# jopohl/urh

Hardware: AMD Instinct MI355X
Metric: Msamples/s IQ->bits (1 GiB complex64 2-FSK per GPU, qad materialised, compact outputs copied to the host) (higher is better)
Workload: dtype f32

## Files before the change

include/urhgpu.h:

```cpp
#ifndef URHGPU_H
#define URHGPU_H

#include <stdint.h>

#ifdef __cplusplus
extern "C" {
#endif

#define URHGPU_VERSION 100

#define URHGPU_OK 0
#define URHGPU_ERR_HIP (-1)
#define URHGPU_ERR_DTYPE (-2)
#define URHGPU_ERR_ARG (-3)
#define URHGPU_ERR_CAPACITY (-4)
#define URHGPU_ERR_UNSUPPORTED (-5)
#define URHGPU_ERR_NO_DEVICE (-6)

#define URHGPU_DT_I8 0
#define URHGPU_DT_U8 1
#define URHGPU_DT_I16 2
#define URHGPU_DT_U16 3
#define URHGPU_DT_F32 4

// ... 216 lines not shown
int urhgpu_msg_divisor_histogram(const uint64_t *lens, int64_t n, uint64_t *hist_out, int64_t cap, int64_t *hist_len, int64_t *tol_out);
int urhgpu_bit_length_from_order(const uint64_t *hist, const int64_t *order_desc, int64_t len, int64_t *bitlen_out);

int urhgpu_minmax(urhgpu_ctx *ctx, const void *arr, int dtype, int64_t n, void *out2);
int urhgpu_segment_messages(urhgpu_ctx *ctx, const void *magnitudes, int is_f64, int64_t n, float noise_threshold, int64_t *seg_out,
                            int64_t cap_seg, int64_t *n_seg);
int urhgpu_get_plateau_lengths(urhgpu_ctx *ctx, const float *rect_data, int64_t n, float center, int percentage, uint64_t *out, int64_t cap,
                               int64_t *n_out);
int urhgpu_threshold_divisor_histogram(const uint64_t *lens, int64_t n, float threshold, uint64_t *hist_out, int64_t cap, int64_t *hist_len);
int urhgpu_median_filter(urhgpu_ctx *ctx, const double *data, int64_t n, unsigned int k, float *out);

int urhgpu_test_fast_division_dev(urhgpu_ctx *ctx, uint64_t seed, int reps, uint64_t *n_mismatch);
int urhgpu_test_sincosf_fast_dev(urhgpu_ctx *ctx, uint64_t *n_mismatch);
int urhgpu_test_force_merge_ambiguous(int on);

int urhgpu_modulate_dev(urhgpu_ctx *ctx, const uint8_t *bits, const int64_t *bit_off, const uint32_t *pause, const uint32_t *start,
                        int n_msgs, uint32_t samples_per_symbol, int mod, const float *parameters, int bits_per_symbol,
                        float carrier_amplitude, float carrier_frequency, float carrier_phase, float sample_rate, int dtype,
                        void *d_out, int64_t cap_samples, int64_t *total_samples);
int urhgpu_modulate(urhgpu_ctx *ctx, const uint8_t *bits, int64_t num_bits, uint32_t samples_per_symbol, int mod,
                    const float *parameters, int bits_per_symbol, float carrier_amplitude, float carrier_frequency,
                    float carrier_phase, float sample_rate, uint32_t pause, uint32_t start, int dtype, void *out);

int urhgpu_modulate_gfsk_dev(urhgpu_ctx *ctx, const uint8_t *bits, const int64_t *bit_off, const uint32_t *pause, const uint32_t *start,
                             int n_msgs, uint32_t samples_per_symbol, const float *parameters, int bits_per_symbol,
                             float carrier_amplitude, float carrier_phase, float sample_rate, int dtype, const float *gauss_fir,
                             int n_taps, const float *frequencies, void *d_out, int64_t cap_samples, int64_t *total_samples);
int urhgpu_modulate_gfsk(urhgpu_ctx *ctx, const uint8_t *bits, int64_t num_bits, uint32_t samples_per_symbol, const float *parameters,
                         int bits_per_symbol, float carrier_amplitude, float carrier_phase, float sample_rate, uint32_t pause,
                         uint32_t start, int dtype, const float *gauss_fir, int n_taps, const float *frequencies, void *out);

int urhgpu_convert_dev(urhgpu_ctx *ctx, const void *d_src, int src_dtype, void *d_dst, int dst_dtype, int64_t n);
int urhgpu_pcm_to_iq_dev(urhgpu_ctx *ctx, const void *d_raw, int64_t n_frames, int channels, int sample_width, float *d_out);
int urhgpu_fft_peak_dev(urhgpu_ctx *ctx, const float *d_x, int64_t n, int64_t *peak_index);
int urhgpu_sub_encode_runs(const uint8_t *values, int64_t n, int64_t stride, int64_t *runs_out, int64_t cap, int64_t *n_runs);
int urhgpu_astype_dev(urhgpu_ctx *ctx, const void *d_src, int src_dtype, void *d_dst, int dst_dtype, int64_t n);

int urhgpu_path_minmax_dev(urhgpu_ctx *ctx, const void *d_samples, int dtype, int64_t start, int64_t end,
                           int64_t samples_per_pixel, void *d_values);
int urhgpu_path_minmax(urhgpu_ctx *ctx, const void *samples, int dtype, int64_t n, int64_t start, int64_t end,
                       int64_t samples_per_pixel, void *values);

int urhgpu_spectrogram_dev(urhgpu_ctx *ctx, const float *d_x, int64_t n, int window_size, int64_t hop, int64_t frames,
                           const double *d_window, const double *d_twiddles, double *d_stft, float *d_db);
int urhgpu_bgra_lookup_dev(urhgpu_ctx *ctx, const float *d_db, int64_t frames, int window_size, const uint32_t *d_colormap,
                           int n_colors, float data_min, float data_max, uint32_t *d_image);

int urhgpu_bench_copy_ceiling_dev(urhgpu_ctx *ctx, const float *d_in, float *d_out, int64_t n_samples, int shape, int reps, float *ms_per_copy);
int urhgpu_test_hot_probe(urhgpu_ctx *ctx, const void *d_iq, int64_t n, const urhgpu_params *p, float *d_qad, int stream_kind, int event_mode,
                          int graded, int launches, int keep, void *d_chunks_out, int64_t *n_chunks_out, float *dur_ms, float *gap_ms, int bubble_us,
                          int load_kind);
int urhgpu_test_hot_stamps(int on);
int urhgpu_test_tail_skip(int mask);
int urhgpu_test_fetch_chunk_tables(urhgpu_ctx *ctx, void *host_dst, int64_t n_chunks);
int urhgpu_memcpy_to_host(urhgpu_ctx *ctx, const void *d_src, void *host_dst, int64_t bytes);
int urhgpu_memcpy_dtod(urhgpu_ctx *ctx, void *d_dst, const void *d_src, int64_t bytes);

int urhgpu_test_force_state_bytes(int on);

int urhgpu_test_force_generic_tail(int on);

int urhgpu_test_force_tiles_per_chunk(int tiles);

int64_t urhgpu_test_wide_int_launches(void);

int64_t urhgpu_test_costas_host_syncs(void);
int64_t urhgpu_test_center_host_syncs(void);
int urhgpu_test_costas_scratch(int64_t n, int loop_order, int64_t *out3);

int urhgpu_test_atan2f_dev(urhgpu_ctx *ctx, const float *d_y, const float *d_x, int64_t n, float *d_out);

int urhgpu_chunk_power_stats_dev(urhgpu_ctx *ctx, const void *d_src, int dtype, int64_t n_rows, void *d_dst, int64_t n_store, double *sum_out,
                                 double *max_out);
int urhgpu_chunk_stats_launches(urhgpu_ctx *ctx, int64_t *n_launches);

int urhgpu_magnitude_chunk_partials_dev(urhgpu_ctx *ctx, const void *d_iq, int dtype, int64_t n_local, int64_t pos_base, int64_t n_total,
                                        int64_t chunk, int64_t n_chunks, double *d_sum, double *d_max);
#define URHGPU_PW_REC_HEAD 8
#define URHGPU_PW_REC_FIRST 136
#define URHGPU_PW_REC_LAST 264
#define URHGPU_PW_REC_TAIL 392
#define URHGPU_PW_REC_PIECES 520
int urhgpu_pairwise_partial_f32_dev(urhgpu_ctx *ctx, const float *d_x, int64_t m_local, int64_t g_off, int64_t m_total, int mode, float mean,
                                    float *d_out, int64_t cap, int64_t *n_out);

typedef struct urhgpu_noise_result {
    double noise;
    float noise_f32;
    float noise_sqrd;
    int64_t flag;
    int64_t chunk, n_chunks;
    int64_t n_candidates;
    double min_mean, max_mean;
} urhgpu_noise_result;
double urhgpu_noise_max_magnitude(int dtype);
int urhgpu_detect_noise_level_dev(urhgpu_ctx *ctx, const void *d_iq, int dtype, int64_t n, void *d_result);
int urhgpu_iq_to_bits_auto_dev(urhgpu_ctx *ctx, const void *d_iq, int64_t n, const urhgpu_params *p, int auto_noise, int auto_center,
                               int64_t center_max_size, const urhgpu_outputs *out, void *d_noise_result, void *h_noise_result,
                               void *d_center_result, void *h_center_result, int64_t hist_cap);
int urhgpu_stream_set_auto_noise(urhgpu_stream *st, int enable);
int urhgpu_stream_noise(urhgpu_stream *st, int64_t seq, double *noise, int64_t *flag);
int64_t urhgpu_test_noise_host_syncs(void);

typedef struct urhgpu_msg_record {
    double rssi;
    int64_t first_pos;
// ... 15 lines not shown
```

urh_amd/_lib.py:

```python
import ctypes as C
import os
import threading

HERE = os.path.dirname(os.path.abspath(__file__))
LIB_PATH = os.path.join(HERE, "liburhgpu.so")

OK = 0
ERR_HIP, ERR_DTYPE, ERR_ARG, ERR_CAPACITY, ERR_UNSUPPORTED, ERR_NO_DEVICE = -1, -2, -3, -4, -5, -6
BLOB_LEN16 = 2
BLOB_ROW16 = 4

DT_I8, DT_U8, DT_I16, DT_U16, DT_F32 = 0, 1, 2, 3, 4
MOD_ASK, MOD_FSK, MOD_PSK, MOD_OTHER = 0, 1, 2, 3
ROW_ABSORBED = -(1 << 62)
BLOB_MAGIC = 0x55524842424C4F42
BLOB_HEADER_BYTES = 128


class UrhGpuError(RuntimeError):
    def __init__(self, status, msg):
        super().__init__(msg)
        self.status = status


# ... 95 lines not shown
    "urhgpu_test_noise_host_syncs": (_i64, []),
    "urhgpu_msg_records_dev": (_i, [_vp, _vp, _i64, C.POINTER(Params), C.POINTER(Outputs), _i64, _vp, _i64, _vp]),
    "urhgpu_stream_set_msg_records": (_i, [_vp, _i, _i64]),
    "urhgpu_stream_msg_records": (_i, [_vp, _i64, C.POINTER(_vp), C.POINTER(_i64)]),
    "urhgpu_test_records_host_syncs": (_i64, []),
    "urhgpu_blob_capacity": (_i64, [_i64, _i64, _i64, _i64, _i]),
    "urhgpu_outputs_to_host": (_i, [_vp, C.POINTER(Outputs), _i, _vp, _i64, C.POINTER(_i64)]),
    "urhgpu_host_libm_check": (_i, [C.POINTER(_i64)]),
    "urhgpu_stream_capacities": (_i, [_i64, C.POINTER(Params), C.POINTER(_i64), C.POINTER(_i64), C.POINTER(_i64), C.POINTER(_i64)]),
    "urhgpu_stream_create": (_i, [_vp, _i64, C.POINTER(Params), _i, _i, _i64, C.POINTER(_vp)]),
    "urhgpu_stream_destroy": (_i, [_vp]),
    "urhgpu_stream_push": (_i, [_vp, _vp, _i64, C.POINTER(HostResult)]),
    "urhgpu_stream_push_upload": (_i, [_vp, _vp, _vp, _i64, C.POINTER(HostResult)]),
    "urhgpu_stream_flush": (_i, [_vp, C.POINTER(HostResult), C.POINTER(_i)]),
    "urhgpu_stream_stats": (_i, [_vp, C.POINTER(_i64)]),
    "urhgpu_stream_wide_passes": (_i, [_vp, C.POINTER(_i64)]),
    "urhgpu_stream_costas_stats": (_i, [_vp, C.POINTER(_i64)]),
    "urhgpu_shard_runs_dev": (_i, [_vp, _vp, _i64, _i64, _i64, _i, _i, _vp, C.POINTER(Params), C.POINTER(Outputs), _vp]),
    "urhgpu_shard_prelaunch_dev": (_i, [_vp, _vp, _i64, _i64, _i64, _i, _i, C.POINTER(Params), C.POINTER(Outputs)]),
    "urhgpu_shard_launch_dev": (_i, [_vp, _vp, _i64, _i64, _i64, _i, _i, _vp, C.POINTER(Params), C.POINTER(Outputs)]),
    "urhgpu_shard_rows_dev": (_i, [_vp, _vp, _vp]),
    "urhgpu_shard_bits_prepare_dev": (_i, [_vp, _vp, _vp]),
    "urhgpu_shard_bits_finish_dev": (_i, [_vp, _vp]),
    "urhgpu_costas_halo_samples": (_i64, [C.POINTER(Params)]),
    "urhgpu_shard_costas_spec_dev": (_i, [_vp, _vp, _i64, _i64, _i64, _i, _i, _vp, _i64, C.POINTER(Params), C.POINTER(Outputs), _vp]),
    "urhgpu_shard_costas_resolve_dev": (_i, [_vp, C.POINTER(C.c_uint32), _vp]),
    "urhgpu_magnitude_chunk_stats_dev": (_i, [_vp, _vp, _i, _i64, _i64, _i64, _vp, _vp]),
    "urhgpu_segment_runs_dev": (_i, [_vp, _vp, _i, _i64, _f, _vp, _i64, _vp]),
    "urhgpu_message_ranges_dev": (_i, [_vp, _vp, _i, _i64, _f, _vp, _i64, C.POINTER(_i64), _vp, _i64, C.POINTER(_i64), C.POINTER(_i)]),
    "urhgpu_message_ranges_demod_dev": (_i, [_vp, _vp, _i, _i64, _f, _vp, _i64, C.POINTER(_i64), _vp, _i64, C.POINTER(_i64), C.POINTER(_i), _vp]),
    "urhgpu_compact_gt_dev": (_i, [_vp, _vp, _i64, _f, _vp, _vp]),
    "urhgpu_edges_le_dev": (_i, [_vp, _vp, _i64, _f, _vp, _i64, _vp]),
    "urhgpu_minmax_f32_dev": (_i, [_vp, _vp, _i64, _vp]),
    "urhgpu_pairwise_sum_f32_dev": (_i, [_vp, _vp, _i64, _i, _f, C.POINTER(_f)]),
    "urhgpu_histogram_f32_dev": (_i, [_vp, _vp, _i64, _vp, _i64, _vp]),
    "urhgpu_msg_center_stats": (_i, [_vp, _vp, _i64, _vp, _i, _i64, _vp, _vp, _vp, _vp]),
    "urhgpu_msg_plateaus": (_i, [_vp, _vp, _i64, _vp, _vp, _i, _i, _i64, _vp, _vp, _i64]),
    "urhgpu_detect_modulation_dev": (_i, [_vp, _vp, _i64, _vp, _i, _i, _i, _vp, _vp]),
    "urhgpu_msg_bit_lengths": (_i, [_vp, _vp, _i, _vp, _vp]),
    "urhgpu_msg_plateau_decisions": (_i, [_vp, _vp, _i64, _vp, _vp, _i, _i, _i64, _vp, _vp]),
    "urhgpu_msg_estimate": (_i, [_vp, _vp, _i64, _vp, _i, _i64, _i, _i64, _vp, _vp, _vp, _vp, _vp]),
    "urhgpu_test_bit_length_from_counts": (_i, [_vp, _i64, C.POINTER(_i64), C.POINTER(_i64)]),
    "urhgpu_msg_divisor_histogram": (_i, [_vp, _i64, _vp, _i64, C.POINTER(_i64), C.POINTER(_i64)]),
    "urhgpu_bit_length_from_order": (_i, [_vp, _vp, _i64, C.POINTER(_i64)]),
    "urhgpu_merge_plateaus": (_i, [_vp, _i64, C.c_uint64, C.c_uint64, _vp, C.POINTER(_i64)]),
    "urhgpu_minmax": (_i, [_vp, _vp, _i, _i64, _vp]),
    "urhgpu_segment_messages": (_i, [_vp, _vp, _i, _i64, _f, _vp, _i64, C.POINTER(_i64)]),
    "urhgpu_get_plateau_lengths": (_i, [_vp, _vp, _i64, _f, _i, _vp, _i64, C.POINTER(_i64)]),
    "urhgpu_threshold_divisor_histogram": (_i, [_vp, _i64, _f, _vp, _i64, C.POINTER(_i64)]),
    "urhgpu_median_filter": (_i, [_vp, _vp, _i64, C.c_uint, _vp]),
    "urhgpu_test_hot_probe": (_i, [_vp, _vp, _i64, C.POINTER(Params), _vp, _i, _i, _i, _i, _i, _vp, C.POINTER(_i64), _vp, _vp, _i, _i]),
    "urhgpu_test_hot_stamps": (_i, [_i]),
    "urhgpu_test_tail_skip": (_i, [_i]),
    "urhgpu_test_fetch_chunk_tables": (_i, [_vp, _vp, _i64]),
    "urhgpu_test_fast_division_dev": (_i, [_vp, C.c_uint64, _i, C.POINTER(C.c_uint64)]),
    "urhgpu_test_sincosf_fast_dev": (_i, [_vp, C.POINTER(C.c_uint64)]),
    "urhgpu_test_force_merge_ambiguous": (_i, [_i]),
    "urhgpu_modulate_dev": (_i, [_vp, _vp, _vp, _vp, _vp, _i, C.c_uint32, _i, _vp, _i, _f, _f, _f, _f, _i, _vp, _i64, C.POINTER(_i64)]),
    "urhgpu_modulate": (_i, [_vp, _vp, _i64, C.c_uint32, _i, _vp, _i, _f, _f, _f, _f, C.c_uint32, C.c_uint32, _i, _vp]),
    "urhgpu_modulate_gfsk_dev": (_i, [_vp, _vp, _vp, _vp, _vp, _i, C.c_uint32, _vp, _i, _f, _f, _f, _i, _vp, _i, _vp, _vp, _i64, C.POINTER(_i64)]),
    "urhgpu_modulate_gfsk": (_i, [_vp, _vp, _i64, C.c_uint32, _vp, _i, _f, _f, _f, C.c_uint32, C.c_uint32, _i, _vp, _i, _vp, _vp]),
    "urhgpu_spectrogram_dev": (_i, [_vp, _vp, _i64, _i, _i64, _i64, _vp, _vp, _vp, _vp]),
    "urhgpu_bgra_lookup_dev": (_i, [_vp, _vp, _i64, _i, _vp, _i, _f, _f, _vp]),
    "urhgpu_convert_dev": (_i, [_vp, _vp, _i, _vp, _i, _i64]),
    "urhgpu_pcm_to_iq_dev": (_i, [_vp, _vp, _i64, _i, _i, _vp]),
    "urhgpu_sub_encode_runs": (_i, [_vp, _i64, _i64, _vp, _i64, _vp]),
    "urhgpu_fft_peak_dev": (_i, [_vp, _vp, _i64, _vp]),
    "urhgpu_astype_dev": (_i, [_vp, _vp, _i, _vp, _i, _i64]),
    "urhgpu_path_minmax_dev": (_i, [_vp, _vp, _i, _i64, _i64, _i64, _vp]),
    "urhgpu_path_minmax": (_i, [_vp, _vp, _i, _i64, _i64, _i64, _i64, _vp]),
    "urhgpu_bench_copy_ceiling_dev": (_i, [_vp, _vp, _vp, _i64, _i, _i, C.POINTER(_f)]),
    "urhgpu_memcpy_to_host": (_i, [_vp, _vp, _vp, _i64]),
    "urhgpu_memcpy_dtod": (_i, [_vp, _vp, _vp, _i64]),
    "urhgpu_test_force_state_bytes": (_i, [_i]),
    "urhgpu_test_force_tiles_per_chunk": (_i, [_i]),
    "urhgpu_test_wide_int_launches": (_i64, []),
    "urhgpu_test_costas_host_syncs": (_i64, []),
    "urhgpu_test_costas_scratch": (_i, [_i64, _i, C.POINTER(_i64)]),
    "urhgpu_test_force_generic_tail": (_i, [_i]),
    "urhgpu_test_atan2f_dev": (_i, [_vp, _vp, _vp, _i64, _vp]),
    "urhgpu_chunk_power_stats_dev": (_i, [_vp, _vp, _i, _i64, _vp, _i64, C.POINTER(C.c_double), C.POINTER(C.c_double)]),
    "urhgpu_chunk_stats_launches": (_i, [_vp, C.POINTER(_i64)]),
    "urhgpu_magnitude_chunk_partials_dev": (_i, [_vp, _vp, _i, _i64, _i64, _i64, _i64, _i64, _vp, _vp]),
    "urhgpu_pairwise_partial_f32_dev": (_i, [_vp, _vp, _i64, _i64, _i64, _i, _f, _vp, _i64, C.POINTER(_i64)]),
}

_lib = None
_lock = threading.Lock()


def _share_torch_hip_runtime():
    import importlib.util
    try:
        spec = importlib.util.find_spec("torch")
    except (ImportError, ValueError):
        spec = None
    if spec is None or not spec.origin:
        return
    cand = os.path.join(os.path.dirname(spec.origin), "lib", "libamdhip64.so")
    if os.path.exists(cand):
        try:
            C.CDLL(cand, mode=C.RTLD_GLOBAL)
        except OSError:
            pass


# ... 133 lines not shown
```

urh_amd/csrc/common.hpp:

```cpp
#pragma once
#include <hip/hip_runtime.h>
#include <stdint.h>
#include <stdio.h>
#include <string.h>

#include <atomic>
#include <vector>

#include "../../include/urhgpu.h"

#ifndef URH_TAIL_PRIO_LEVEL
#define URH_TAIL_PRIO_LEVEL 3
#endif
#ifndef URH_TAIL_PAD
#define URH_TAIL_PAD 0
#endif
#if URH_TAIL_PAD
#define URH_TAIL_PRIO() do { __builtin_amdgcn_s_setprio(URH_TAIL_PRIO_LEVEL); __asm__ volatile("v_mov_b32 v95, 0" ::: "v95"); } while (0)
#else
#define URH_TAIL_PRIO() __builtin_amdgcn_s_setprio(URH_TAIL_PRIO_LEVEL)
#endif

namespace urh {

// ... 51 lines not shown

constexpr size_t kSmallPinned = size_t(1) << 20;
constexpr int kNoiseMaxChunks = 199;
constexpr size_t kNoiseWorkBytes = 128 * 1024;
struct urhgpu_ctx {
    int device = 0;
    hipStream_t own_stream = nullptr;
    hipStream_t stream = nullptr;
    hipDeviceProp_t prop;
    urh::Arena arena;
    urh::Arena staging;
    urh::Arena aux;
    urh::Arena fir_work;
    hipEvent_t ev_fir = nullptr;
    hipStream_t fir_stream = nullptr;
    int64_t *d_counts = nullptr;
    int64_t *h_counts = nullptr;
    bool tune_spin_wait = true;
    bool tune_wide_int = false;
    bool tune_shard_summary_generic = false;
    int tune_costas_dev_rounds = -1;
    int32_t *costas_stats_next = nullptr;
    hipStream_t last_tail = nullptr;
    int wide_int_next = 0;
    char *h_small = nullptr;
    int32_t *d_tickets = nullptr;
    void *d_desc = nullptr;
    size_t desc_cap = 0;
    void *d_rdesc = nullptr;
    size_t rdesc_cap = 0;
    unsigned long long scan_epoch = 0x0ACE0FBA5E000000ull;
    std::vector<hipEvent_t> prof_events;
    std::vector<bool> prof_dispatch;
    int prof_used = 0;
    bool prof_on = false;
    bool prof_bracket = false;
    void *shard = nullptr;
    bool pipelined = false;
    int hot_lds_pad_sharded = 33 * 1024;
    int tune_hot_cus_removed = 4;
    hipStream_t hot_masked = nullptr;
    hipEvent_t ev_in = nullptr;
    int hot_lds_pad = 0;
    hipStream_t tail_stream = nullptr;
    bool own_tail_stream = false;
    urh::Arena arena_alt, arena_alt2;
    hipEvent_t ev_hot = nullptr;
    hipEvent_t ev_tail[3] = {nullptr, nullptr, nullptr};
    int flip = 0;
    bool tail_pending = false;
    int tile_parity = 0;
    void *d_seg = nullptr;
    bool seg_dirty[3] = {false, false, false};
    int tune_stream_segments = 7;
    int tune_stream_policy = 5;
    long long passes_begun = 0;
    bool tune_stream_latency = false;
    bool tune_stream_pos_direct = true;
    int tune_upload_pieces = 4;
    hipEvent_t ev_piece[16] = {};
    hipEvent_t ev_hot_done[3] = {nullptr, nullptr, nullptr};
    hipStream_t bits_stream = nullptr;
    hipEvent_t ev_rows[3][16] = {};
    hipEvent_t ev_bits[3] = {nullptr, nullptr, nullptr};
    urh::Arena chunk_work;
    double *h_chunk = nullptr;
    long long chunk_launches = 0;
    urh::Arena center_work;
    int tune_center_max_bins = 4096;
    hipEvent_t ev_center = nullptr;
    void *d_noise_work = nullptr;
    int wide_int_auto = 0;
};
constexpr size_t kSegBlockBytes = 4096;

namespace urh {
int iq_to_bits_streamed(urhgpu_ctx *ctx, const void *d_iq, int64_t n, const urhgpu_params *p, const urhgpu_outputs *out, void *host_blob,
                        int64_t cap_host, hipEvent_t ev_ready, bool *streamed, const void *h_iq, void *stage_blob = nullptr, bool *staged = nullptr,
                        hipEvent_t ev_rows = nullptr, int len16 = 0);
hipError_t wait_stream(const urhgpu_ctx *ctx, hipStream_t s);
int reserve_psk_pass(urhgpu_ctx *ctx, int64_t n_max, int tolerance, bool want_qad);
int join_tail(urhgpu_ctx *ctx);
inline int stage_in(urhgpu_ctx *ctx, const void *host, size_t bytes, void **dev) {
    void *d = ctx->staging.take(bytes ? bytes : 16);
    if (!d) return URHGPU_ERR_ARG;
    if (bytes) URH_HIP(hipMemcpyAsync(d, host, bytes, hipMemcpyHostToDevice, ctx->stream));
    *dev = d;
    return URHGPU_OK;
}
inline int fetch_out(urhgpu_ctx *ctx, void *host, const void *dev, size_t bytes) {
    URH_HIP(hipMemcpyAsync(host, dev, bytes, hipMemcpyDeviceToHost, ctx->stream));
    URH_HIP(hipStreamSynchronize(ctx->stream));
    return URHGPU_OK;
}
}
```

urh_amd/csrc/compact.hpp:

```cpp
#pragma once
#include <stdint.h>

#include "../../include/urhgpu.h"

namespace urh {

struct BlobLayout {
    int64_t n_rows, n_msg, n_bits, n_pos;
    int64_t off_pauses, off_msg_off, off_pos_off, off_row_state, off_bits, off_row_len, off_pos32, total;
};

__host__ __device__ inline BlobLayout blob_layout(const int64_t *counts5, int64_t cap_rows, int64_t cap_bits, int64_t cap_msg, int64_t cap_pos,
                                                  int has_pos) {
    BlobLayout L;
    L.n_rows = counts5[0] < cap_rows ? counts5[0] : cap_rows;
    L.n_msg = counts5[1] < cap_msg ? counts5[1] : cap_msg;
    L.n_bits = counts5[2] < cap_bits ? counts5[2] : cap_bits;
    L.n_pos = has_pos ? (counts5[3] < cap_pos ? counts5[3] : cap_pos) : 0;
    if (L.n_rows < 0) L.n_rows = 0;
    if (L.n_msg < 0) L.n_msg = 0;
    if (L.n_bits < 0) L.n_bits = 0;
    if (L.n_pos < 0) L.n_pos = 0;
    auto up = [](int64_t x) { return (x + 15) & ~int64_t(15); };
    int64_t o = URHGPU_BLOB_HEADER_BYTES;
    L.off_pauses = o; o = up(o + L.n_msg * 8);
    L.off_msg_off = o; o = up(o + (L.n_msg + 1) * 8);
    L.off_pos_off = o; o = up(o + (L.n_msg + 1) * 8);
    L.off_row_state = o; o = up(o + L.n_rows);
    L.off_bits = o; o = up(o + (L.n_bits + 7) / 8);
    L.off_row_len = o; o = up(o + L.n_rows * 4);
    L.off_pos32 = o; o = up(o + L.n_pos * 4);
    L.total = o;
    return L;
}

struct StagedLayout { int64_t head_cap, off_row_state, off_row_len, off_pos32, total; };
__host__ __device__ inline StagedLayout staged_layout(int64_t cap_rows, int64_t cap_bits, int64_t cap_msg, int64_t cap_pos, int has_pos) {
    const int64_t c[5] = {0, cap_msg, cap_bits, 0, 0};
    auto up = [](int64_t x) { return (x + 15) & ~int64_t(15); };
    StagedLayout S;
    S.head_cap = blob_layout(c, cap_rows, cap_bits, cap_msg, cap_pos, 0).total;
    S.off_row_state = S.head_cap;
    S.off_row_len = up(S.off_row_state + cap_rows);
    S.off_pos32 = up(S.off_row_len + 4 * cap_rows);
    S.total = up(S.off_pos32 + (has_pos ? 4 * cap_pos : 0));
    return S;
}

inline int64_t blob_capacity(int64_t cap_rows, int64_t cap_bits, int64_t cap_msg, int64_t cap_pos, int has_pos) {
    const int64_t c[5] = {cap_rows, cap_msg, cap_bits, cap_pos, cap_rows};
    return blob_layout(c, cap_rows, cap_bits, cap_msg, cap_pos, has_pos).total;
}

}
```

urh_amd/csrc/ctx.hip:

```cpp
#include <chrono>

#include "pass.hpp"
#include "fdlibm_atan2f.h"
#include "glibc_sincosf.h"

namespace urh {

thread_local char g_hip_err[256] = "";
std::atomic<long long> g_center_host_syncs{0};
thread_local int g_center_scope = 0;
std::atomic<long long> g_noise_host_syncs{0};
thread_local int g_noise_scope = 0;
std::atomic<long long> g_records_host_syncs{0};
thread_local int g_records_scope = 0;

int Arena::reserve(size_t bytes) {
    if (bytes <= cap) return URHGPU_OK;
    if (base) { center_note_wait(); URH_HIP(hipFree(base)); base = nullptr; cap = 0; }
    const size_t want = (bytes + (size_t(1) << 20)) & ~((size_t(1) << 20) - 1);
    URH_HIP(hipMalloc(&base, want));
    cap = want;
    used = 0;
    return URHGPU_OK;
}
// ... 58 lines not shown
    hipError_t e = hipGetDeviceCount(&c);
    if (e != hipSuccess) { *count = 0; (void)hipGetLastError(); return URHGPU_ERR_NO_DEVICE; }
    *count = c;
    return URHGPU_OK;
}

int urhgpu_ctx_create(int device, urhgpu_ctx **out) {
    if (!out) return URHGPU_ERR_ARG;
    int c = 0;
    if (urhgpu_device_count(&c) != URHGPU_OK || c <= 0 || device < 0 || device >= c) return URHGPU_ERR_NO_DEVICE;
    urhgpu_ctx *ctx = new (std::nothrow) urhgpu_ctx();
    if (!ctx) return URHGPU_ERR_ARG;
    ctx->device = device;
    URH_HIP(hipSetDevice(device));
    URH_HIP(hipGetDeviceProperties(&ctx->prop, device));
    URH_HIP(hipStreamCreateWithFlags(&ctx->own_stream, hipStreamNonBlocking));
    ctx->stream = ctx->own_stream;
    URH_HIP(hipMalloc((void **)&ctx->d_counts, 16 * sizeof(int64_t)));
    URH_HIP(hipMalloc((void **)&ctx->d_tickets, 16 * sizeof(int32_t)));
    URH_HIP(hipMemset(ctx->d_tickets, 0, 16 * sizeof(int32_t)));
    URH_HIP(hipMalloc(&ctx->d_noise_work, kNoiseWorkBytes));
    {
        const int32_t aux0[4] = {kAuxNone, kAuxNone, kAuxNone, -1};
        URH_HIP(hipMemcpy(ctx->d_tickets + 4, aux0, sizeof(aux0), hipMemcpyHostToDevice));
    }
    URH_HIP(hipHostMalloc((void **)&ctx->h_counts, 32 * sizeof(int64_t)));
    memset(ctx->h_counts, 0, 32 * sizeof(int64_t));
    if (hipHostMalloc((void **)&ctx->h_small, kSmallPinned) != hipSuccess) { (void)hipGetLastError(); ctx->h_small = nullptr; }
    *out = ctx;
    return URHGPU_OK;
}

int urhgpu_ctx_destroy(urhgpu_ctx *ctx) {
    if (!ctx) return URHGPU_OK;
    (void)hipSetDevice(ctx->device);
    (void)hipStreamSynchronize(ctx->stream);
    ctx->arena.release();
    ctx->staging.release();
    ctx->aux.release();
    ctx->fir_work.release();
    ctx->chunk_work.release();
    ctx->center_work.release();
    if (ctx->ev_center) (void)hipEventDestroy(ctx->ev_center);
    if (ctx->h_chunk) (void)hipHostFree(ctx->h_chunk);
    if (ctx->ev_fir) (void)hipEventDestroy(ctx->ev_fir);
    ctx->arena_alt.release();
    ctx->arena_alt2.release();
    if (ctx->hot_masked) { (void)hipStreamSynchronize(ctx->hot_masked); (void)hipStreamDestroy(ctx->hot_masked); }
    if (ctx->ev_in) (void)hipEventDestroy(ctx->ev_in);
    if (ctx->tail_stream) (void)hipStreamSynchronize(ctx->tail_stream);
    if (ctx->own_tail_stream && ctx->tail_stream) (void)hipStreamDestroy(ctx->tail_stream);
    if (ctx->d_seg) {
        (void)hipFree(ctx->d_seg);
        if (ctx->bits_stream) { (void)hipStreamSynchronize(ctx->bits_stream); (void)hipStreamDestroy(ctx->bits_stream); }
        for (hipEvent_t e : ctx->ev_piece) if (e) (void)hipEventDestroy(e);
        for (int k = 0; k < 3; ++k) {
            if (ctx->ev_hot_done[k]) (void)hipEventDestroy(ctx->ev_hot_done[k]);
            if (ctx->ev_bits[k]) (void)hipEventDestroy(ctx->ev_bits[k]);
            for (hipEvent_t e : ctx->ev_rows[k]) if (e) (void)hipEventDestroy(e);
        }
    }
    if (ctx->ev_hot) { (void)hipEventDestroy(ctx->ev_hot); (void)hipEventDestroy(ctx->ev_tail[0]); (void)hipEventDestroy(ctx->ev_tail[1]); (void)hipEventDestroy(ctx->ev_tail[2]); }
    free_shard_session(ctx);
    for (hipEvent_t e : ctx->prof_events) (void)hipEventDestroy(e);
    if (ctx->d_counts) (void)hipFree(ctx->d_counts);
    if (ctx->d_tickets) (void)hipFree(ctx->d_tickets);
    if (ctx->d_noise_work) (void)hipFree(ctx->d_noise_work);
    if (ctx->d_desc) (void)hipFree(ctx->d_desc);
    if (ctx->d_rdesc) (void)hipFree(ctx->d_rdesc);
    if (ctx->h_counts) (void)hipHostFree(ctx->h_counts);
    if (ctx->h_small) (void)hipHostFree(ctx->h_small);
    if (ctx->own_stream) (void)hipStreamDestroy(ctx->own_stream);
    delete ctx;
    return URHGPU_OK;
}

int urhgpu_ctx_set_stream(urhgpu_ctx *ctx, void *hip_stream) {
    if (!ctx) return URHGPU_ERR_ARG;
    ctx->stream = (hipStream_t)hip_stream;
    return URHGPU_OK;
}

int urhgpu_ctx_use_private_stream(urhgpu_ctx *ctx) {
    if (!ctx) return URHGPU_ERR_ARG;
    ctx->stream = ctx->own_stream;
    return URHGPU_OK;
}

int urhgpu_ctx_sync(urhgpu_ctx *ctx) {
    if (!ctx) return URHGPU_ERR_ARG;
    if (ctx->hot_masked) URH_HIP(hipStreamSynchronize(ctx->hot_masked));
    if (ctx->bits_stream) URH_HIP(hipStreamSynchronize(ctx->bits_stream));
    if (ctx->tail_stream) URH_HIP(hipStreamSynchronize(ctx->tail_stream));
    URH_HIP(hipStreamSynchronize(ctx->stream));
    ctx->tail_pending = false;
    return URHGPU_OK;
}

int urhgpu_ctx_set_pipelined(urhgpu_ctx *ctx, int enable, void *tail_stream) {
    if (!ctx) return URHGPU_ERR_ARG;
    URH_HIP(hipSetDevice(ctx->device));
    URH_TRY(urhgpu_ctx_sync(ctx));
    if (ctx->own_tail_stream && ctx->tail_stream) { (void)hipStreamDestroy(ctx->tail_stream); }
    ctx->tail_stream = nullptr; ctx->own_tail_stream = false; ctx->pipelined = false;
    if (ctx->hot_masked) { (void)hipStreamSynchronize(ctx->hot_masked); (void)hipStreamDestroy(ctx->hot_masked); ctx->hot_masked = nullptr; }
    if (!enable) return URHGPU_OK;
    if (tail_stream) ctx->tail_stream = (hipStream_t)tail_stream;
    else {
        URH_HIP(hipStreamCreateWithFlags(&ctx->tail_stream, hipStreamNonBlocking));
        ctx->own_tail_stream = true;
    }
    if (!ctx->ev_hot) {
        URH_HIP(hipEventCreateWithFlags(&ctx->ev_hot, hipEventDisableTiming));
        for (hipEvent_t &e : ctx->ev_tail) URH_HIP(hipEventCreateWithFlags(&e, hipEventDisableTiming));
    }
    if (ctx->tune_hot_cus_removed > 0 && ctx->prop.multiProcessorCount == 256) {
        const int words = 8;
        uint32_t mask[8];
        hot_cu_mask(ctx->tune_hot_cus_removed, mask);
        if (hipExtStreamCreateWithCUMask(&ctx->hot_masked, (uint32_t)words, mask) != hipSuccess) { (void)hipGetLastError(); ctx->hot_masked = nullptr; }
        if (ctx->hot_masked && !ctx->ev_in && hipEventCreateWithFlags(&ctx->ev_in, hipEventDisableTiming) != hipSuccess) {
            (void)hipGetLastError();
            (void)hipStreamDestroy(ctx->hot_masked);
            ctx->hot_masked = nullptr;
        }
    }
    ctx->pipelined = true;
    return URHGPU_OK;
}

int urhgpu_ctx_set_tuning(urhgpu_ctx *ctx, const char *key, int value) {
    if (!ctx || !key) return URHGPU_ERR_ARG;
    if (!strcmp(key, "hot_lds_kb")) { if (value < 0 || value > 150) return URHGPU_ERR_ARG; ctx->hot_lds_pad = value * 1024; }
    else if (!strcmp(key, "hot_lds_kb_sharded")) { if (value < 0 || value > 150) return URHGPU_ERR_ARG; ctx->hot_lds_pad_sharded = value * 1024; }
    else if (!strcmp(key, "profile_bracket")) ctx->prof_bracket = value != 0;
    else if (!strcmp(key, "hot_cus_removed_per_xcd")) { if (value < 0 || value > 16) return URHGPU_ERR_ARG; ctx->tune_hot_cus_removed = value; }
    else if (!strcmp(key, "stream_segments")) { if (value < 1 || value > kMaxSegments) return URHGPU_ERR_ARG; ctx->tune_stream_segments = value; }
    else if (!strcmp(key, "stream_policy")) { if (value < 0 || value > 6) return URHGPU_ERR_ARG; ctx->tune_stream_policy = value; }
    else if (!strcmp(key, "stream_latency")) { ctx->tune_stream_latency = value != 0; }
    else if (!strcmp(key, "stream_pos_direct")) { ctx->tune_stream_pos_direct = value != 0; }
    else if (!strcmp(key, "spin_wait")) { ctx->tune_spin_wait = value != 0; }
    else if (!strcmp(key, "shard_summary_generic")) { ctx->tune_shard_summary_generic = value != 0; }
    else if (!strcmp(key, "wide_int")) { ctx->tune_wide_int = value != 0; }
    else if (!strcmp(key, "costas_dev_rounds")) { if (value < -1 || value > 24) return URHGPU_ERR_ARG; ctx->tune_costas_dev_rounds = value; }
    else if (!strcmp(key, "upload_pieces")) { if (value < 2 || value > kMaxSegments) return URHGPU_ERR_ARG; ctx->tune_upload_pieces = value; }
    else if (!strcmp(key, "auto_center_max_bins")) { if (value < 1 || value > (1 << 20)) return URHGPU_ERR_ARG; ctx->tune_center_max_bins = value; }
    else return URHGPU_ERR_ARG;
    return URHGPU_OK;
}

int urhgpu_ctx_join(urhgpu_ctx *ctx) {
    if (!ctx) return URHGPU_ERR_ARG;
    URH_HIP(hipSetDevice(ctx->device));
    return join_tail(ctx);
}

int urhgpu_host_libm_check(int64_t *out4) {
    if (!out4) return URHGPU_ERR_ARG;
    static const uint32_t kDiscriminating[17] = {0x418a3adbu, 0x418a3adcu, 0x418a3addu, 0x418a3adeu, 0x41bc76d9u, 0x4202eb4bu, 0x4255b0a9u, 0x4280ce28u,
                                                 0x42687a55u, 0x42a35c07u, 0x42a35d44u, 0x42870e40u, 0x42a97360u, 0x42c55faau, 0x42d8d23eu, 0x42e87a55u,
                                                 0x42cf5854u};
    int64_t n_sc = 0, bad_sc = 0, n_at = 0, bad_at = 0;
    auto same = [](float a, float b) { uint32_t x, y; memcpy(&x, &a, 4); memcpy(&y, &b, 4); return x == y || (a != a && b != b); };
    auto check_sc = [&](float x) {
        volatile float vx = x;
        n_sc += 2;
        if (!same(sinf(vx), urh_sinf(x))) ++bad_sc;
        if (!same(cosf(vx), urh_cosf(x))) ++bad_sc;
    };
    for (uint32_t u : kDiscriminating) {
        float x; memcpy(&x, &u, 4);
        check_sc(x); check_sc(-x);
    }
    uint64_t s = 0x243f6a8885a308d3ull;
    auto next = [&]() { s += 0x9e3779b97f4a7c15ull; uint64_t z = s; z = (z ^ (z >> 30)) * 0xbf58476d1ce4e5b9ull; z = (z ^ (z >> 27)) * 0x94d049bb133111ebull; return z ^ (z >> 31); };
    for (int i = 0; i < 4096; ++i) {
        const uint64_t z = next();
        check_sc((float)((double)(int64_t)(z >> 11) * (1.0 / 9007199254740992.0) * 240.0 - 120.0));
        const uint32_t a = (uint32_t)z, b = (uint32_t)(z >> 32);
        float y, x;
        const uint32_t uy = (a & 0x807fffffu) | (((a >> 23) % 41u + 107u) << 23), ux = (b & 0x807fffffu) | (((b >> 23) % 41u + 107u) << 23);
        memcpy(&y, &uy, 4); memcpy(&x, &ux, 4);
        volatile float vy = y, vx = x;
        ++n_at;
        if (!same(atan2f(vy, vx), urh_atan2f(y, x))) ++bad_at;
    }
    out4[0] = n_sc; out4[1] = bad_sc; out4[2] = n_at; out4[3] = bad_at;
    return URHGPU_OK;
}

int urhgpu_ctx_info(urhgpu_ctx *ctx, int *compute_units, int *wavefront, int64_t *hbm_bytes, char *name, int name_cap) {
    if (!ctx) return URHGPU_ERR_ARG;
// ... 84 lines not shown
```

urh_amd/csrc/demod_runs.hip:

```cpp
#include <atomic>
#include <hip/hip_runtime.h>
#include <hip/hip_ext.h>

#include <algorithm>

#include "cmul.hpp"
#include "common.hpp"
#include "fdlibm_atan2f.h"
#include "launchers.hpp"
#include "runs.hpp"

namespace urh {

enum { SRC_IQ = 0, SRC_QAD = 1 };

#ifndef URH_KBATCH
#define URH_KBATCH 2
#endif
#ifndef URH_MINWAVES
#define URH_MINWAVES 1
#endif
#ifndef URH_SPEC
#ifndef URH_WIDE_INT
#define URH_WIDE_INT 0
// ... 1349 lines not shown
    {
        int o = incl - cnt;
        const int64_t base = p.pos_base + a0 + (int64_t)lane * kRowSamples;
        while (ae | ao) {
            const int pos = bp_first(ae, ao);
            const uint64_t rec = rec_make(base + pos, state_at(pos));
            if (through) __hip_atomic_store(slab + o, rec, __ATOMIC_RELAXED, __HIP_MEMORY_SCOPE_AGENT);
            else slab[o] = rec;
            ++o;
            if (pos & 1) ao &= ao - 1; else ae &= ae - 1;
        }
    }
    const uint64_t am = __builtin_amdgcn_ballot_w64(cnt > 0);
    uint32_t first_state = 0xFFFFu; int64_t last_pos = 0;
    if (am) {
        const int fl = __builtin_ctzll(am), ll = 63 - __builtin_clzll(am);
        first_state = __builtin_amdgcn_readlane(first_acc_state, fl);
        last_pos = p.pos_base + a0 + (int64_t)ll * kRowSamples + __builtin_amdgcn_readlane(last_acc, ll);
    }
    const uint32_t last_state = hm ? (uint32_t)__builtin_amdgcn_readlane(my_last, 63 - __builtin_clzll(hm)) : 0xFFFFu;

    if (lane == 0) {
        ChunkInfo ci;
        ci.pend_pos = (pend_pos >= 0) ? pend_pos + p.pos_base : -1;
        ci.start = p.pos_base + a0;
        ci.len = a1 - a0;
        ci.lead = lead;
        ci.cnt = total;
        ci.first_state = (uint16_t)first_state;
        ci.last_state = (uint16_t)last_state;
        ci.pend_state = (uint16_t)pend_state;
        ci.last_pos = last_pos;
        ci.init_state = (uint16_t)chunk_init_state<SRC, DT, MOD, NPL == 1>(p, chunk);
        ci.first_acc = 0; ci.pend_acc = 0; ci.pend_stable = 0; ci.pad = 0;
        if (STAMPS) {
            const unsigned hw = __builtin_amdgcn_s_getreg((4 ) | (0 << 6) | (31 << 11));
            const unsigned xcc = __builtin_amdgcn_s_getreg((20 ) | (0 << 6) | (3 << 11));
            ci.first_acc = p.chunks[chunk].first_acc; ci.pend_stable = p.chunks[chunk].pend_stable; ci.pad = (int32_t)(uint32_t)wall_clock64();
            ci.pend_acc = (int32_t)((hw & 0xFFFFu) | ((xcc & 0xFu) << 16));
        }
        if (through) {
            static_assert(sizeof(ChunkInfo) % 8 == 0, "ChunkInfo is written as 64-bit words");
            uint64_t w[sizeof(ChunkInfo) / 8];
            __builtin_memcpy(w, &ci, sizeof(ChunkInfo));
            uint64_t *dst = (uint64_t *)(p.chunks + chunk);
#pragma unroll
            for (int k = 0; k < (int)(sizeof(ChunkInfo) / 8); ++k) __hip_atomic_store(dst + k, w[k], __ATOMIC_RELAXED, __HIP_MEMORY_SCOPE_AGENT);
        } else {
            p.chunks[chunk] = ci;
        }
    }
    if (through) {
        __asm__ volatile("s_waitcnt vmcnt(0)" ::: "memory");
        if (lane == 0) {
            int k = 0;
            while (k < p.n_seg - 1 && chunk >= (int64_t)p.seg_end[k]) ++k;
            __hip_atomic_fetch_add(p.progress + k * kProgressStride, 1u, __ATOMIC_RELAXED, __HIP_MEMORY_SCOPE_AGENT);
        }
    }
}

constexpr int kAfpBlock = 256;
constexpr int kAfpRow = kAfpBlock * 2;

template <int DT, int MOD, bool DNOISE = false>
__global__ __launch_bounds__(kAfpBlock) void k_afp_demod(const RunArgs p) {
    const int lane = threadIdx.x & 63;
    const float nsq = DNOISE ? *p.d_noise : 0.f;
    const bool global_start = (p.left_halo == nullptr);
    const int64_t stride = (int64_t)gridDim.x * kAfpRow;
    for (int64_t base = (int64_t)blockIdx.x * kAfpRow; base < p.n; base += stride) {
        const int64_t i0 = base + 2 * threadIdx.x;
        float c0 = 0, d0 = 0, c1 = 0, d1 = 0;
        const bool v1 = (i0 + 1 < p.n), v0 = (i0 < p.n);
        if (v1) Iq<DT>::load2(p.in, i0, c0, d0, c1, d1);
        else if (v0) Iq<DT>::load1(p.in, i0, c0, d0);
        float sc = 0, sd = 0;
        if (MOD == URHGPU_MOD_FSK) {
            const int64_t w0 = base + 2 * (threadIdx.x - lane);
            if (w0 >= 1) { if (w0 - 1 < p.n) Iq<DT>::load1(p.in, w0 - 1, sc, sd); }
            else if (!global_start) Iq<DT>::load1(p.left_halo, 1, sc, sd);
        }
        const float pc = dpp_wave_shr1(c1, sc), pd = dpp_wave_shr1(d1, sd);
        if (v0) {
            float q0 = demod_one<MOD, URHGPU_DT_F32, DNOISE>(pc, pd, c0, d0, p, nsq);
            if (i0 == 0 && global_start) q0 = p.noise_val;
            if (v1) {
                const float q1 = demod_one<MOD, URHGPU_DT_F32, DNOISE>(c0, d0, c1, d1, p, nsq);
                *(float2 *)(p.qad + i0) = make_float2(q0, q1);
            } else {
                p.qad[i0] = q0;
            }
        }
    }
}
__global__ void k_test_div(uint64_t seed, int reps, unsigned long long *mismatches) {
    uint64_t s = seed + (blockIdx.x * (uint64_t)blockDim.x + threadIdx.x) * 0x9e3779b97f4a7c15ull;
    unsigned long long bad = 0;
    for (int i = 0; i < reps; ++i) {
        s += 0x9e3779b97f4a7c15ull;
        uint64_t z = s; z = (z ^ (z >> 30)) * 0xbf58476d1ce4e5b9ull; z = (z ^ (z >> 27)) * 0x94d049bb133111ebull; z ^= z >> 31;
        const uint32_t a = (uint32_t)z, b = (uint32_t)(z >> 32);
        const float d = __uint_as_float(((b % 80u + 87u) << 23) | (b >> 9));
        const float f = __uint_as_float((a & 0x807fffffu) | 0x3f000000u);
        const float n = f * d * __uint_as_float((97u + (a >> 23) % 57u) << 23);
        float q2, q3;
        div_fast2(n, d, d * 0.25f, n == 0.f ? 1.0f : n * 8.0f, q2, q3);
        const float q1 = n / d;
        if (__float_as_uint(q1) != __float_as_uint(q2)) ++bad;
        if (__float_as_uint(div_fast(n, d)) != __float_as_uint(q1)) ++bad;
// ... 218 lines not shown
```

urh_amd/csrc/launchers.hpp:

```cpp
#pragma once
#include <atomic>
#include <hip/hip_runtime.h>
#include <stdint.h>

#include "common.hpp"
#include "runs.hpp"

namespace urh {

struct RunArgs {
    const void *in;
    float *qad;
    const void *left_halo;
    int64_t n;
    int64_t range_begin;
    int64_t range_end;
    int64_t chunk_base;
    int64_t pos_base;
    int64_t chunk_len;
    uint64_t *slab;
    int64_t slab_stride;
    ChunkInfo *chunks;
    float noise_sqrd;
    float noise_val;
    float max_magnitude;
    int order;
    int tol;
    int launch_part;
    int seg_mode;
    float dm_noise_sqrd, dm_max_magnitude, dm_noise_val;
    int lds_pad;
    uint32_t *progress;
    int32_t n_seg;
    int32_t seg_end[kMaxSegments];
    int64_t launch_lo, launch_hi;
    int64_t graded_from, graded_len;
    int wide_int;
    int stamp_probe;
    float thr[kMaxOrder - 1];
    const float *d_thr;
    const float *d_noise;
};
extern bool g_force_state_bytes;
extern std::atomic<long long> g_wide_int_launches;
extern bool g_stamp_probe;
extern int g_tail_skip;
struct HotEvents { hipEvent_t start = nullptr, stop = nullptr; bool used = false; };
int launch_wide_probe(const void *d_iq, int dtype, int64_t n, float noise_sqrd, int32_t *h_out, hipStream_t s, const float *d_noise = nullptr);
int launch_demod_runs_iq(const RunArgs &a, int dtype, int mod, bool write_qad, hipStream_t s, HotEvents *ev = nullptr);
int launch_runs_qad(const RunArgs &a, hipStream_t s, HotEvents *ev = nullptr);
bool runs_streamable(const RunArgs &a);
int launch_afp_demod(const RunArgs &a, int dtype, int mod, int grid, hipStream_t s);
void launch_test_div(uint64_t seed, int reps, unsigned long long *d_mismatches, hipStream_t s);
void launch_test_sincosf_fast(unsigned long long *d_mismatches, hipStream_t s);
void launch_test_atan2f(const float *y, const float *x, int64_t n, float *out, hipStream_t s);

struct ModMsg {
    int64_t bit_off;
    int64_t n_sym;
    int64_t sym_off;
    int64_t out_off;
    uint32_t pause;
    uint32_t start;
};
constexpr int kModGfsk = 5;
struct ModArgs {
    const uint8_t *bits;
    const ModMsg *msgs;
    const float *params;
    float *phase;
    void *out;
    int n_msgs, mod, dtype, bps;
    int oqpsk;
    const float *taps;
    int n_taps;
    int freq_given;
    float *gf_freq, *gf_phase;
    uint32_t sps;
    float carrier_amplitude, carrier_frequency, carrier_phase, sample_rate;
};
int launch_modulate(const ModArgs &a, int64_t max_samples, hipStream_t s);

int launch_stft(const float2 *x, int64_t n, int ws, int64_t hop, int64_t frames, const double *window, const double2 *tw,
                double2 *out_c128, float *out_db, hipStream_t s);
int launch_bgra_lookup(const float *data, int64_t frames, int ws, const uint32_t *colormap, int n_colors, float dmin, float dmax,
                       uint32_t *image, hipStream_t s);
// ... 92 lines not shown
size_t merge_scratch_bytes(int64_t cap);
int launch_merge_rows_ask(const int64_t *rows_in, const int64_t *d_n_in, int64_t cap, int64_t *rows_out,
                          int64_t cap_out, int64_t *d_n_out, void *scratch, int32_t *tickets, hipStream_t s);
size_t bits_scratch_bytes(int64_t cap_rows);
struct ScanState {
    int32_t *tickets;
    void *desc;
    size_t desc_bytes;
    unsigned long long *epoch;
};
size_t bits_desc_bytes(int64_t cap_rows);
int launch_ppseq_to_bits(const int64_t *rows, const int64_t *d_n_rows, int64_t cap_rows, const BitsParams &bp,
                         const BitsOut &o, void *scratch, const ScanState &ss, hipStream_t s);
int launch_bits_prepare(const int64_t *rows, const int64_t *d_n_rows, int64_t cap_rows, const BitsParams &bp,
                        void *scratch, int64_t *d_flags, const ScanState &ss, hipStream_t s);
int launch_bits_finish(const int64_t *rows, const int64_t *d_n_rows, int64_t cap_rows, const BitsParams &bp,
                       const BitsOut &o, void *scratch, const ScanState &ss, hipStream_t s);
struct SegState {
    int64_t rows_at[kMaxSegments];
    int64_t rows_needed;
    int64_t n_acc;
    int64_t n_groups;
    int64_t n_groups_local;
    int64_t end_bits, end_pos, end_msgs;
    int64_t err;
    struct In {
        int64_t g0;
        int64_t carry[3];
        int64_t ship_bits, ship_pos, ship_msgs, pad;
    } in[2];
};
static_assert(sizeof(SegState) == 128 + 64 + 128, "SegState");
constexpr int64_t kSegAlign = 256;
struct SegGate {
    const uint32_t *progress;
    int k;
    uint32_t target;
    int init;
    SegState *seg;
    long long max_ticks;
    int fused;
};
struct RowsSegment {
    int index;
    int final;
    int64_t c0, c1;
    SegGate gate;
    int8_t *h_state;
    int32_t *h_len;
    int fuse_gate;
    int len16;
    int64_t *esc;
    int64_t esc_cap;
};
struct BitsSegment {
    int index;
    int final;
    int64_t c0, c1;
    int rows_index;
    SegState *state;
};
struct SegPackDst {
    void *host;
    int64_t cap_host;
    uint32_t *progress_reset;
    int blocks;
    int pos_direct;
    int split;
    void *host_head;
    const int64_t *esc;
    int64_t esc_cap;
    int64_t row16_esc_off;
};

struct TileTailMem {
    void *mem;
    int64_t n_chunks;
    int32_t *huge_count;
    int parity;
    void *rdesc;
    unsigned long long epoch;
    int64_t *d_row_base = nullptr;
};
size_t tile_rdesc_bytes(int64_t n_chunks);
size_t tile_tail_bytes(int64_t n_chunks);
int64_t tile_desc_cap(int64_t cap_rows, int64_t n_chunks);
int launch_tile_rows(const ResolveArgs &r, const EmitArgs &e, const TileTailMem &m, const BitsParams *bp, hipStream_t s);
int launch_tile_bits(const TileTailMem &m, const int64_t *rows, const int64_t *d_n_rows, int64_t cap_rows, const BitsParams &bp,
                     const BitsOut &o, void *scratch, const ScanState &ss, hipStream_t s);
int launch_tile_bits_prepare(const TileTailMem &m, const int64_t *rows, const int64_t *d_n_rows, int64_t cap_rows, const BitsParams &bp,
                             void *scratch, int64_t *d_flags, const ScanState &ss, hipStream_t s);
int launch_tile_bits_finish(const TileTailMem &m, const int64_t *rows, const int64_t *d_n_rows, int64_t cap_rows, const BitsParams &bp,
                            const BitsOut &o, void *scratch, const ScanState &ss, hipStream_t s);
int launch_rows_segment(const ResolveArgs &r, const EmitArgs &e, const TileTailMem &m, const BitsParams &bp, SegState *state, const RowsSegment &sg,
                        hipStream_t s);
int launch_bits_segment(const TileTailMem &m, const BitsParams &bp, const BitsOut &o, void *scratch, const ScanState &ss, int64_t *rows,
                        int64_t cap_rows, const BitsSegment &sg, const SegPackDst *dst, hipStream_t s);
void launch_merge_summary(const int64_t *rows, const int64_t *d_n_rows, int64_t *d_out5, hipStream_t s);
void launch_merge_fix(int64_t *rows, const int64_t *d_n_rows, const int64_t *d_all, int rank, int world,
                      int64_t *d_absorbed, hipStream_t s);
void launch_bits_extra(const int64_t *d_all, int rank, int world, int32_t *d_extra, hipStream_t s);

size_t fir_stats_scratch_bytes(int64_t n);
size_t fir_work_bytes(int64_t n, int m);
int launch_fir(const float2 *x, int64_t n, const float2 *taps, int m, const float2 *halo, float2 *out, hipStream_t s, void *work = nullptr,
               int64_t chunk = 0, int64_t n_chunks = 0, double *d_sum = nullptr, double *d_max = nullptr, void *tile_scratch = nullptr);
int launch_iir(const double *a, int64_t M, const double *b, int64_t N, const float2 *x, int64_t n, float2 *y, hipStream_t s);
int launch_magnitudes(const void *iq, int dtype, int64_t n, double *out, hipStream_t s);
size_t mag_chunk_scratch_bytes(int64_t n_chunks);
int launch_mag_chunk_stats(const void *iq, int dtype, int64_t n, int64_t chunk, int64_t n_chunks, double *d_sum, double *d_max,
                           void *scratch, hipStream_t s);
int launch_noise_chain(const void *iq, int dtype, int64_t n, double max_mag, float cfg_noise, int use_cfg, void *work, void *d_result, void *h_result,
                       hipStream_t s);
size_t compact_scratch_bytes(int64_t n);
int launch_compact_gt(const float *x, int64_t n, const int64_t *d_n, float thr, float *out, int64_t *d_count, void *scratch,
                      int32_t *tickets, hipStream_t s);
int launch_compact_edges(const float *x, int64_t n, const int64_t *d_n, float center, int64_t *out, int64_t cap, int64_t *d_count,
                         void *scratch, int32_t *tickets, hipStream_t s);
size_t minmax_scratch_bytes();
int launch_minmax(const float *x, int64_t n, float *d_out2, void *scratch, hipStream_t s);
int launch_minmax_any(const void *x, int dtype, int64_t n, void *d_out2, void *scratch, hipStream_t s);
int launch_above_flags(const void *mag, int is_f64, int64_t n, float thr, float *flags, hipStream_t s);
int launch_median_filter(const double *data, int64_t n, int k, float *out, hipStream_t s);
constexpr int kDtAboveFlags = 100;
int pairwise_sum_f32(urhgpu_ctx *ctx, const float *d_x, int64_t n, int mode, float mean, float *out);
// ... 40 lines not shown
```

urh_amd/csrc/probes.hip:

```cpp
#include "pass.hpp"

using namespace urh;

#define URH_PROBE_WPB 4

namespace urh {
bool g_tile_tail = true;
int g_force_tiles_per_chunk = 0;
}

extern "C" {

int urhgpu_test_fast_division_dev(urhgpu_ctx *ctx, uint64_t seed, int reps, uint64_t *n_mismatch) {
    if (!ctx || !n_mismatch || reps < 0) return URHGPU_ERR_ARG;
    URH_HIP(hipSetDevice(ctx->device));
    URH_HIP(hipMemsetAsync(ctx->d_counts, 0, 8, ctx->stream));
    launch_test_div(seed, reps, (unsigned long long *)ctx->d_counts, ctx->stream);
    URH_HIP(hipGetLastError());
    URH_TRY(fetch_out(ctx, ctx->h_counts, ctx->d_counts, 8));
    *n_mismatch = (uint64_t)ctx->h_counts[0];
    return URHGPU_OK;
}

int urhgpu_test_force_merge_ambiguous(int on) {
// ... 16 lines not shown
int urhgpu_bench_copy_ceiling_dev(urhgpu_ctx *ctx, const float *d_in, float *d_out, int64_t n_samples, int shape, int reps, float *ms_per_copy) {
    if (!ctx || !d_in || !d_out || !ms_per_copy || n_samples < 8192 || n_samples % 8192 || reps < 1 || shape < 0 || shape > 2) return URHGPU_ERR_ARG;
    if (((uintptr_t)d_in & 15) || ((uintptr_t)d_out & 15)) return URHGPU_ERR_ARG;
    URH_HIP(hipSetDevice(ctx->device));
    URH_TRY(urhgpu_ctx_sync(ctx));
    hipStream_t cs = ctx->stream;
    if (shape == 2) {
        if (!ctx->hot_masked) return URHGPU_ERR_UNSUPPORTED;
        cs = ctx->hot_masked; shape = 0;
    }
    hipEvent_t e0, e1;
    URH_HIP(hipEventCreate(&e0));
    URH_HIP(hipEventCreate(&e1));
    for (int k = 0; k < 3; ++k) launch_copy_shape(d_in, d_out, n_samples, shape, cs);
    URH_HIP(hipEventRecord(e0, cs));
    for (int k = 0; k < reps; ++k) launch_copy_shape(d_in, d_out, n_samples, shape, cs);
    URH_HIP(hipEventRecord(e1, cs));
    URH_HIP(hipEventSynchronize(e1));
    float ms = 0.f;
    URH_HIP(hipEventElapsedTime(&ms, e0, e1));
    (void)hipEventDestroy(e0); (void)hipEventDestroy(e1);
    *ms_per_copy = ms / (float)reps;
    return URHGPU_OK;
}

__global__ void k_probe_valu(long long ticks, int prio, float *sink) {
    if (prio) __builtin_amdgcn_s_setprio(3);
    const long long t0 = (long long)wall_clock64();
    float x = (float)threadIdx.x, y = 1.0f;
    unsigned long long z = threadIdx.x;
    do {
#pragma unroll
        for (int k = 0; k < 64; ++k) { x = x * 1.0001f + y; y = y * 0.9999f + x; z = z * 6364136223846793005ull + 1442695040888963407ull; }
    } while ((long long)wall_clock64() - t0 < ticks);
    if (x == 12345.678f && z == 42) *sink = y;
}
__global__ void k_probe_latency(long long ticks, const unsigned long long *mem, unsigned long long lines, unsigned long long *sink) {
    const long long t0 = (long long)wall_clock64();
    unsigned long long at = (blockIdx.x * 256ull + threadIdx.x) * 0x9e3779b97f4a7c15ull, acc = 0;
    do {
#pragma unroll 1
        for (int k = 0; k < 8; ++k) { const unsigned long long v = mem[(at % lines) * 8]; acc += v; at = at * 6364136223846793005ull + v + 1442695040888963407ull; }
    } while ((long long)wall_clock64() - t0 < ticks);
    if (acc == 0x1234567ull) *sink = acc;
}

__global__ void k_probe_spin(long long ticks) {
    const long long t0 = (long long)wall_clock64();
    while ((long long)wall_clock64() - t0 < ticks) __builtin_amdgcn_s_sleep(16);
}

int urhgpu_test_hot_stamps(int on) { urh::g_stamp_probe = (on != 0); return URHGPU_OK; }
int urhgpu_test_tail_skip(int mask) { urh::g_tail_skip = mask; return URHGPU_OK; }

int urhgpu_test_fetch_chunk_tables(urhgpu_ctx *ctx, void *host_dst, int64_t n_chunks) {
    if (!ctx || !host_dst || n_chunks < 1) return URHGPU_ERR_ARG;
    URH_HIP(hipSetDevice(ctx->device));
    URH_TRY(urhgpu_ctx_sync(ctx));
    const size_t bytes = (size_t)n_chunks * sizeof(ChunkInfo);
    const urh::Arena *order[3] = {&ctx->arena, &ctx->arena_alt2, &ctx->arena_alt};
    for (int k = 0; k < 3; ++k) {
        if (!order[k]->base || order[k]->cap < bytes) { memset((char *)host_dst + k * bytes, 0, bytes); continue; }
        URH_HIP(hipMemcpy((char *)host_dst + k * bytes, order[k]->base, bytes, hipMemcpyDeviceToHost));
    }
    return URHGPU_OK;
}

int urhgpu_test_hot_probe(urhgpu_ctx *ctx, const void *d_iq, int64_t n, const urhgpu_params *p, float *d_qad, int stream_kind, int event_mode,
                          int graded, int launches, int keep, void *d_chunks_out, int64_t *n_chunks_out, float *dur_ms, float *gap_ms, int bubble_us,
                          int load_kind) {
    if (!ctx || !d_iq || !p || !d_qad || !d_chunks_out || !n_chunks_out || launches < 1 || keep < 1 || keep > launches || n < kTile || n % kTile) return URHGPU_ERR_ARG;
    if (p->dtype != URHGPU_DT_F32 || p->mod != URHGPU_MOD_FSK || p->bits_per_symbol != 1) return URHGPU_ERR_UNSUPPORTED;
    URH_HIP(hipSetDevice(ctx->device));
    URH_TRY(join_tail(ctx));
    URH_TRY(urhgpu_ctx_sync(ctx));
    const Plan pl = make_plan(ctx, n, p->tolerance);
    const int64_t g = std::min<int64_t>(std::max(graded, 0), pl.n_chunks);
    const int64_t short_len = pl.chunk_len / 4;
    if (g > 0 && ((short_len % (URH_PROBE_WPB * kRowSamples)) != 0 || n % pl.chunk_len != 0)) return URHGPU_ERR_UNSUPPORTED;
    const int64_t n_launch = pl.n_chunks + 3 * g;
    URH_TRY(ctx->arena.reserve((size_t)n_launch * sizeof(ChunkInfo) + (size_t)n_launch * pl.slab_stride * 8 + 4096));
    ctx->arena.reset();
    ChunkInfo *chunks = (ChunkInfo *)ctx->arena.take((size_t)n_launch * sizeof(ChunkInfo));
    uint64_t *slab = (uint64_t *)ctx->arena.take((size_t)n_launch * pl.slab_stride * 8);
    if (!chunks || !slab) return URHGPU_ERR_ARG;
    RunArgs a;
    URH_TRY(hot_run_args(ctx, p, pl, n, 0, true, &a));
    a.in = d_iq; a.qad = d_qad; a.wide_int = 0;
    a.chunks = chunks; a.slab = slab; a.stamp_probe = 1;
    if (g > 0) { a.graded_from = pl.n_chunks - g; a.graded_len = short_len; }
    hipStream_t s = ctx->stream;
    if (stream_kind == 1) { if (!ctx->hot_masked) return URHGPU_ERR_UNSUPPORTED; s = ctx->hot_masked; }
    std::vector<hipEvent_t> ev((size_t)launches * 2, nullptr);
    if (event_mode != 0) {
        const unsigned fl = event_mode == 1 ? hipEventDisableTiming : event_mode == 2 ? (hipEventDisableTiming | hipEventDisableSystemFence | hipEventReleaseToDevice) : hipEventDefault;
        for (auto &e : ev) URH_HIP(hipEventCreateWithFlags(&e, fl));
    }
    hipStream_t s2 = nullptr;
    void *load_mem = nullptr;
    if (load_kind != 0) {
        if (event_mode == 0 || event_mode == 3) return URHGPU_ERR_ARG;
        if (load_kind == 3 || load_kind == 5) URH_HIP(hipStreamCreateWithFlags(&s2, hipStreamNonBlocking));
        else {
            uint32_t m[8], inv[8];
            hot_cu_mask(ctx->tune_hot_cus_removed, m);
            for (int w = 0; w < 8; ++w) inv[w] = ~m[w];
// ... 59 lines not shown
```

urh_amd/csrc/pulse_table.hip:

```cpp
#include <hip/hip_runtime.h>

#include <algorithm>

#include "common.hpp"
#include "compact.hpp"
#include "launchers.hpp"
#include "runs.hpp"
#include "scan.hpp"

namespace urh {

#ifndef URH_RESOLVE_BLOCK
#define URH_RESOLVE_BLOCK 256
#endif
#ifndef URH_RESOLVE_ITEMS
#define URH_RESOLVE_ITEMS 4
#endif
constexpr int kResolveBlock = URH_RESOLVE_BLOCK;

__host__ __device__ static inline int64_t resolve_blocks(int64_t n_chunks) { return (n_chunks + kResolveBlock - 1) / kResolveBlock; }

size_t resolve_scratch_bytes(int64_t n_chunks) {
    return (size_t)n_chunks * (4 * 4 + 2 * 8) + (size_t)(resolve_blocks(n_chunks) + 1) * (4 + 4 + 8) + 10 * 256;
}
// ... 847 lines not shown
constexpr int kEmitWaves = 4;
#ifndef URH_TAIL_CPW
#define URH_TAIL_CPW 4
#endif
constexpr int kTailCPW = URH_TAIL_CPW;
#ifndef URH_EXPAND_PREFETCH
#define URH_EXPAND_PREFETCH 1
#endif
#ifndef URH_PACK_WORDS
#define URH_PACK_WORDS 1
#endif
#ifndef URH_EXPAND_EARLY_EXIT
#define URH_EXPAND_EARLY_EXIT 1
#endif
#ifdef URH_TAIL_CAP80
#define URH_TAIL_OCC __attribute__((amdgpu_waves_per_eu(URH_TAIL_CAP80)))
#else
#define URH_TAIL_OCC
#endif
#ifdef URH_OCC_EMIT
#define URH_EMIT_OCC __attribute__((amdgpu_waves_per_eu(URH_OCC_EMIT)))
#else
#define URH_EMIT_OCC
#endif
#ifdef URH_OCC_EXPAND
#define URH_EXPAND_OCC __attribute__((amdgpu_waves_per_eu(URH_OCC_EXPAND)))
#else
#define URH_EXPAND_OCC URH_TAIL_OCC
#endif
static_assert(kResolveBlock % kTailCPW == 0 && kTailCPW <= 64, "the chunks of one wavefront share their resolve workgroup");

__device__ __forceinline__ int64_t lane_bcast(int64_t v, int src) {
    const int lo = __builtin_amdgcn_readlane((int)(uint32_t)(uint64_t)v, src), hi = __builtin_amdgcn_readlane((int)(uint32_t)((uint64_t)v >> 32), src);
    return (int64_t)(((uint64_t)(uint32_t)hi << 32) | (uint32_t)lo);
}
__device__ __forceinline__ int lane_bcast(int v, int src) { return __builtin_amdgcn_readlane(v, src); }

struct EmitTileArgs {
    EmitArgs e;
    ResolveArgs r;
    TileTail ft;
    BitsParams bp;
    HugeRef *huge;
    int32_t huge_cap;
    int64_t w0, w_end;
    int final_seg;
    SegState *seg;
    int seg_k;
    int8_t *h_state;
    int32_t *h_len;
    int len16;
    int64_t *esc;
    int64_t esc_cap;
};

__host__ __device__ static inline int64_t tail_waves(int64_t n_items) { return (n_items + kTailCPW - 1) / kTailCPW; }

__device__ __forceinline__ void ship_row(const EmitTileArgs &g, int64_t idx, int64_t state, int64_t len) {
    if (g.len16 == 2) {
        const bool fits = len >= 0 && len < 0x1FFF;
        ((uint16_t *)g.h_len)[idx] = (uint16_t)((((uint32_t)(state + 1) & 7u) << 13) | (fits ? (uint32_t)len : 0x1FFFu));
        if (!fits) {
            const unsigned long long slot = atomicAdd((unsigned long long *)g.esc, 1ull);
            if ((int64_t)slot < g.esc_cap) g.esc[1 + slot] = (int64_t)(((uint64_t)(uint32_t)(int32_t)len << 32) | (uint64_t)(uint32_t)idx);
        }
        return;
    }
    g.h_state[idx] = (int8_t)state;
    if (!g.len16) { g.h_len[idx] = (int32_t)len; return; }
    const bool fits = len >= 0 && len < 0xFFFF;
    ((uint16_t *)g.h_len)[idx] = fits ? (uint16_t)len : (uint16_t)0xFFFF;
    if (!fits) {
        const unsigned long long slot = atomicAdd((unsigned long long *)g.esc, 1ull);
        if ((int64_t)slot < g.esc_cap) g.esc[1 + slot] = (int64_t)(((uint64_t)(uint32_t)(int32_t)len << 32) | (uint64_t)(uint32_t)idx);
    }
}

__global__ __launch_bounds__(64 * kEmitWaves) URH_EMIT_OCC void k_emit_rows_tiles(const EmitTileArgs g) {
    URH_TAIL_PRIO();
    const EmitArgs &a = g.e;
    const ResolveArgs &r = g.r;
    const int lane = threadIdx.x & 63;
    const int64_t w = g.w0 + (int64_t)blockIdx.x * kEmitWaves + __builtin_amdgcn_readfirstlane((int)(threadIdx.x >> 6));
    const int64_t n_cw = g.w_end;
    if (w > n_cw) return;
    const bool totals = (w == n_cw);
    const bool table = (r.n_local != r.n_chunks);
    const int64_t lc0 = a.chunk_first, lc1 = a.chunk_first + r.n_local;
    const int64_t c0 = totals ? (g.final_seg ? r.n_chunks : n_cw * kTailCPW) : w * kTailCPW;
    const int64_t n_before = (totals && g.final_seg) ? resolve_blocks(r.n_chunks) : c0 / kResolveBlock;
    const uint32_t init_state = a.chunks[0].init_state;
    ResElem first = res_identity();
    if (lane < n_before) first = g.ft.btot[lane];
    const int n_mine = totals ? 0 : (int)((r.n_chunks - c0 < kTailCPW) ? r.n_chunks - c0 : kTailCPW);
    ResElem pl_l = res_identity();
    int cnt_l = 0, fl_l = 0, pp_l = 0;
    int64_t pend_pos_l = -1, last_pos_l = 0;
    if (lane < n_mine) {
        pl_l = g.ft.ploc[c0 + lane];
        const ChunkInfo *ch = a.chunks + c0 + lane;
        cnt_l = ch->cnt; pend_pos_l = ch->pend_pos;
        if (table) last_pos_l = ch->last_pos;
        fl_l = (int)((uint32_t)ch->first_state | ((uint32_t)ch->last_state << 16));
        pp_l = (int)((uint32_t)ch->pend_state | ((uint32_t)(ch->pend_stable ? 1 : 0) << 16));
    }
    uint64_t rec = 0;
    if (n_mine > 0 && c0 >= lc0 && c0 < lc1 && lane < a.slab_stride)
        rec = (a.slab + (c0 - lc0) * a.slab_stride)[lane];
    const ResElem init = res_make(init_state, -1, init_state, 0, false, -1, 0);
    const ResElem base = res_combine(init, res_fold_blocks(g.ft.btot, n_before, lane, first));
    int64_t row_base = 0;
    if (table) row_base = res_before_entry(g.ft, init, lc0, r.n_chunks, lane).cnt;
    if (totals) {
        const ResElem pre = base;
        if (!g.final_seg) {
            if (lane == 0) g.seg->rows_at[g.seg_k] = (r.rows != nullptr && pre.cnt > r.cap_rows) ? r.cap_rows : pre.cnt;
            return;
        }
        const int64_t c = r.n_chunks;
        int64_t row_end = pre.cnt;
        if (table && lc1 < r.n_chunks) row_end = res_before_entry(g.ft, init, lc1, r.n_chunks, lane).cnt;
        if (lane == 0) {
            const int64_t P = pre.cnt;
            *r.d_n_acc = P;
            int64_t n_rows = row_end - row_base;
            int64_t o = n_rows;
            VecK<4> v; v.zero();
            int32_t tcnt = 0;
            if (P < r.n_total && r.write_last_row) {
                o = P - row_base;
                n_rows = o + 1;
                tcnt = 1;
                const int64_t fpos = pre.la_valid() ? pre.la_pos : -1;
                const uint32_t fstate = pre.la_valid() ? pre.la_state() : init_state;
                const int64_t len = (P == 0) ? (r.n_total - r.tol) : (r.n_total - 1 - fpos - r.tol);
                if (r.rows != nullptr && o < r.cap_rows) {
                    r.rows[2 * o] = (int64_t)fstate - 1; r.rows[2 * o + 1] = len;
                    if (g.h_state) ship_row(g, o, (int64_t)fstate - 1, len);
                }
                if (g.ft.want_bits) {
                    v = row_value((int64_t)fstate - 1, len, P == 0, g.bp);
                    if (v.v[0] > kHugeBits) {
                        const int slot = atomicAdd(g.ft.huge_count + g.ft.parity, 1);
                        if (slot < g.huge_cap) { g.huge[slot].tile = c; g.huge[slot].row = o; }
                    }
                }
            }
            *r.d_n_rows_needed = n_rows;
            *r.d_n_rows = (r.rows != nullptr && n_rows > r.cap_rows) ? r.cap_rows : n_rows;
            if (g.ft.d_row_base) *g.ft.d_row_base = row_base;
            g.ft.agg[c] = v; g.ft.tile_off[c] = o; g.ft.tile_cnt[c] = tcnt;
        }
        return;
    }
    for (int jc = 0; jc < n_mine; ++jc) {
        const int64_t c = c0 + jc;
        const bool local = (c >= lc0 && c < lc1);
        const uint64_t *slab = a.slab + (c - lc0) * a.slab_stride;
        uint64_t rec_next = 0;
        if (jc + 1 < n_mine && c + 1 >= lc0 && c + 1 < lc1 && lane < a.slab_stride) rec_next = (a.slab + (c + 1 - lc0) * a.slab_stride)[lane];
        ResElem pl;
        pl.cnt = lane_bcast(pl_l.cnt, jc); pl.first_pos = lane_bcast(pl_l.first_pos, jc); pl.la_pos = lane_bcast(pl_l.la_pos, jc);
        pl.meta = (uint64_t)lane_bcast((int64_t)pl_l.meta, jc);
        const int cnt = lane_bcast(cnt_l, jc);
        const uint32_t fl = (uint32_t)lane_bcast(fl_l, jc), pp = (uint32_t)lane_bcast(pp_l, jc);
        const int64_t pend_pos = lane_bcast(pend_pos_l, jc);
        const uint32_t c_first = fl & 0xFFFFu, c_last = fl >> 16, c_pend = pp & 0xFFFFu;
        const int pend_stable = (int)(pp >> 16);
        const ResElem pre = res_combine(base, pl);
// ... 552 lines not shown


int g_tail_skip = 0;
namespace {
constexpr int kTileHugeCap = 8192;
struct TileCarve { TileTail ft; HugeRef *huge; };
TileCarve carve_tile(const TileTailMem &m) {
    TileCarve tc;
    char *p = (char *)m.mem;
    auto take = [&](size_t bytes) { char *r = p; p += (bytes + 255) & ~size_t(255); return r; };
    const int64_t nt = m.n_chunks + 1;
    tc.ft.ploc = (ResElem *)take((size_t)m.n_chunks * sizeof(ResElem));
    tc.ft.btot = (ResElem *)take((size_t)(resolve_blocks(m.n_chunks) + 1) * sizeof(ResElem));
    tc.ft.agg = (VecK<4> *)take((size_t)nt * sizeof(VecK<4>));
    tc.ft.excl = (VecK<4> *)take((size_t)nt * sizeof(VecK<4>));
    tc.ft.tile_off = (int64_t *)take((size_t)nt * 8);
    tc.ft.tile_cnt = (int32_t *)take((size_t)nt * 4);
    tc.ft.d_n_tiles = (int64_t *)take(64);
    tc.huge = (HugeRef *)take((size_t)kTileHugeCap * sizeof(HugeRef));
    tc.ft.huge_count = m.huge_count;
    tc.ft.parity = m.parity;
    tc.ft.want_bits = 0;
    tc.ft.rdesc = (GranDesc *)m.rdesc;
    tc.ft.epoch = m.epoch;
    tc.ft.d_row_base = m.d_row_base;
    tc.ft.esc = nullptr;
    return tc;
}
}

int64_t tile_desc_cap(int64_t cap_rows, int64_t n_chunks) { return std::max<int64_t>(cap_rows, 8 * (n_chunks + 2) + kScanTile); }

size_t tile_rdesc_bytes(int64_t n_chunks) {
    return (size_t)(resolve_blocks(n_chunks) + 2 + (n_chunks + 1 + kScanBlock - 1) / kScanBlock + 2) * sizeof(GranDesc);
}

size_t tile_tail_bytes(int64_t n_chunks) {
    const int64_t nt = n_chunks + 1;
    return (size_t)n_chunks * sizeof(ResElem) + (size_t)(resolve_blocks(n_chunks) + 1) * sizeof(ResElem) + (size_t)nt * (2 * sizeof(VecK<4>) + 12) +
           64 + (size_t)kTileHugeCap * sizeof(HugeRef) + 10 * 256;
}

int launch_tile_rows(const ResolveArgs &r, const EmitArgs &e, const TileTailMem &m, const BitsParams *bp, hipStream_t s) {
    if (r.n_chunks <= 0 || r.local_pass || r.chunk_first != e.chunk_first || r.chunk_first < 0 || r.chunk_first + r.n_local > r.n_chunks ||
        m.n_chunks != r.n_chunks || e.is_ask)
        return URHGPU_ERR_ARG;
    if ((r.n_local != r.n_chunks) != (m.d_row_base != nullptr)) return URHGPU_ERR_ARG;
    TileCarve tc = carve_tile(m);
    EmitTileArgs g;
    g.e = e; g.r = r; g.ft = tc.ft; g.huge = tc.huge; g.huge_cap = kTileHugeCap;
    memset(&g.bp, 0, sizeof(g.bp));
    if (bp) { g.bp = *bp; g.ft.want_bits = 1; }
    const unsigned gb = (unsigned)resolve_blocks(r.n_chunks);
    g.w0 = 0; g.w_end = tail_waves(r.n_chunks); g.final_seg = 1; g.seg = nullptr; g.seg_k = 0; g.h_state = nullptr; g.h_len = nullptr; g.len16 = 0; g.esc = nullptr; g.esc_cap = 0; g.ft.esc = nullptr;
    SegGate no_gate;
    memset(&no_gate, 0, sizeof(no_gate));
    if (!(g_tail_skip & 1)) hipLaunchKernelGGL(k_resolve_one, dim3(gb), dim3(kResolveBlock), 0, s, r, g.ft, (int64_t)0, no_gate);
    if (!(g_tail_skip & 2)) hipLaunchKernelGGL(k_emit_rows_tiles, dim3((unsigned)((tail_waves(r.n_chunks) + 1 + kEmitWaves - 1) / kEmitWaves)), dim3(64 * kEmitWaves), 0, s, g);
    return URHGPU_OK;
}

namespace {
__global__ void k_tile_flags(const int64_t *d_n_rows, const GroupInfo *groups, const int64_t *d_n_groups, int64_t *d_flags) {
    const int64_t n = *d_n_rows, ng = *d_n_groups;
    const int64_t n_l = (n > 0 && ng > 0) ? ng - 1 : 0;
    d_flags[0] = n_l > 0;
    d_flags[1] = (n > 0) && groups[0].data_end > 0;
    d_flags[2] = (n > 0) && (groups[n_l].data_end - (n_l ? groups[n_l - 1].data_end : 0) > 0);
}
}

int launch_tile_bits_prepare(const TileTailMem &m, const int64_t *rows, const int64_t *d_n_rows, int64_t cap_rows, const BitsParams &bp,
                             void *scratch, int64_t *d_flags, const ScanState &ss, hipStream_t s) {
    if (cap_rows <= 0) cap_rows = 1;
    const int64_t nt = m.n_chunks + 1;
    const int64_t cap_desc = tile_desc_cap(cap_rows, m.n_chunks);
    if (ss.desc_bytes < bits_desc_bytes(cap_desc)) return URHGPU_ERR_ARG;
    const TileCarve tc = carve_tile(m);
    const BitsScratch b = carve_bits(scratch, cap_rows);
    const int64_t cap_groups = cap_rows + 1;
    GranDesc *tdesc = (GranDesc *)m.rdesc + resolve_blocks(m.n_chunks) + 2;
    TileScanArgs ta{rows, d_n_rows, tc.ft.agg, tc.ft.tile_off, tc.ft.tile_cnt, tc.ft.excl, b.groups, cap_groups, b.d_n_groups, nt, bp, tdesc,
                    m.epoch, 0, nullptr, 0};
    const unsigned nb_ts = (unsigned)((nt + kScanBlock - 1) / kScanBlock);
    if (!(g_tail_skip & 4)) hipLaunchKernelGGL(k_tile_scan, dim3(nb_ts), dim3(kScanBlock), 0, s, ta);
    if (d_flags) hipLaunchKernelGGL(k_tile_flags, dim3(1), dim3(1), 0, s, d_n_rows, b.groups, b.d_n_groups, d_flags);
    return URHGPU_OK;
}

int launch_tile_bits_finish(const TileTailMem &m, const int64_t *rows, const int64_t *d_n_rows, int64_t cap_rows, const BitsParams &bp,
                            const BitsOut &o, void *scratch, const ScanState &ss, hipStream_t s) {
    if (cap_rows <= 0) cap_rows = 1;
    const int64_t nt = m.n_chunks + 1;
    const int64_t cap_desc = tile_desc_cap(cap_rows, m.n_chunks);
    if (ss.desc_bytes < bits_desc_bytes(cap_desc)) return URHGPU_ERR_ARG;
    const TileCarve tc = carve_tile(m);
    const BitsScratch b = carve_bits(scratch, cap_rows);
    ScanDesc<3> *desc3 = (ScanDesc<3> *)((char *)ss.desc + (((size_t)(scan_blocks(cap_desc) + 1) * sizeof(ScanDesc<4>) + 255) & ~size_t(255)));
    GroupLoad gl{b.groups, b.d_n_groups, bp.d_extra, bp.is_last_rank, bp.write_pos};
    GroupStore gs{gl, b.gout, o.msg_off, o.pauses, o.pos_off, o.pos, o.cap_msg, o.cap_pos};
    BitsCountsFinal fin{d_n_rows, o.msg_off, o.pos_off, o.counts, b.huge_count, bp.d_rows_needed, o.h_counts};
    if (!(g_tail_skip & 8))
        hipLaunchKernelGGL((k_scan_lookback<3, GroupLoad, GroupStore, BitsCountsFinal, kGroupItems>), dim3(scan_grid(b.nbg)), dim3(kScanBlock), 0, s,
                           b.d_n_groups, gl, desc3, b.nbg, gs, fin, ++*ss.epoch, ss.tickets + 2, 0);
    ExpandTileArgs ea{rows, d_n_rows, tc.ft.excl, tc.ft.tile_off, tc.ft.tile_cnt, b.gout, b.d_n_groups, o.bits, o.cap_bits, o.pos, o.cap_pos,
                      bp, tc.huge, m.huge_count, kTileHugeCap, m.parity, nt, 0, nullptr};
    const unsigned tile_blocks = (unsigned)expand_tile_blocks(nt);
// ... 45 lines not shown
    int final;
    BitsCountsFinal counts;
    __device__ void operator()(const VecK<3> &grand) const {
        const SegState::In in = seg->in[parity];
        const int64_t nl = seg->n_groups_local;
        VecK<3> tot;
#pragma unroll
        for (int k = 0; k < 3; ++k) tot.v[k] = in.carry[k] + grand.v[k];
        if (final) {
            counts(tot);
            const bool any = *d_n_rows > 0;
            seg->end_msgs = any ? tot.v[0] : 0; seg->end_bits = any ? tot.v[1] : 0; seg->end_pos = any ? tot.v[2] : 0;
            return;
        }
        SegState::In nx = in;
        if (nl <= 0) {
            seg->end_msgs = 0; seg->end_bits = 0; seg->end_pos = 0;
        } else {
            const int64_t g_open = in.g0 + nl - 1;
            const VecK<3> vo = ld(nl - 1);
            VecK<3> exo;
#pragma unroll
            for (int k = 0; k < 3; ++k) exo.v[k] = tot.v[k] - vo.v[k];
            const int64_t d0 = g_open ? ld.ld.groups[g_open - 1].data_end : 0;
            const bool has_data = ld.ld.groups[g_open].data_end - d0 > 0;
            nx.g0 = g_open;
#pragma unroll
            for (int k = 0; k < 3; ++k) nx.carry[k] = exo.v[k];
            seg->end_msgs = exo.v[0]; seg->end_bits = exo.v[1] + vo.v[1]; seg->end_pos = exo.v[2] + vo.v[2];
            nx.ship_msgs = exo.v[0];
            nx.ship_bits = has_data ? exo.v[1] + vo.v[1] : exo.v[1];
            nx.ship_pos = has_data ? exo.v[2] + vo.v[2] : exo.v[2];
        }
        seg->in[parity ^ 1] = nx;
    }
};

struct SegPack {
    const uint8_t *bits; const int64_t *msg_off, *pauses, *pos_off, *pos; const int64_t *counts;
    int64_t cap_rows, cap_bits, cap_msg, cap_pos;
    int has_pos;
    char *host;
    BlobLayout L;
    const SegState *seg;
    const int64_t *d_n_rows;
    int parity, final;
    uint32_t *progress;
    int pos_shipped;
    int split;
    char *head;
    const int64_t *esc;
    int64_t esc_cap;
    int64_t row16_esc_off;
};
__global__ __launch_bounds__(256) void k_pack_seg(const SegPack a) {
    URH_TAIL_PRIO();
    const int64_t gtid = blockIdx.x * 256ll + threadIdx.x, stride = (int64_t)gridDim.x * 256;
    const SegState::In in = a.seg->in[a.parity];
    auto lim = [](int64_t x, int64_t cap) { return x < cap ? (x < 0 ? 0 : x) : cap; };
    const int64_t nbits = lim(a.seg->end_bits, a.cap_bits);
    const int64_t j0 = lim(in.ship_bits, a.cap_bits) / 8, j1 = a.final ? (nbits + 7) / 8 : nbits / 8;
    const int64_t p0 = a.has_pos ? lim(in.ship_pos, a.cap_pos) : 0, p1 = a.has_pos ? lim(a.seg->end_pos, a.cap_pos) : 0;
    const int64_t m0 = lim(in.ship_msgs, a.cap_msg), m1 = lim(a.seg->end_msgs, a.cap_msg);
    BlobLayout L = a.L;
    if (a.split) {
        const int64_t c5[5] = {0, m1, nbits, 0, 0};
        const BlobLayout T = blob_layout(c5, a.cap_rows, a.cap_bits, a.cap_msg, a.cap_pos, 0);
        L.off_pauses = T.off_pauses; L.off_msg_off = T.off_msg_off; L.off_pos_off = T.off_pos_off; L.off_bits = T.off_bits;
    }
    {
        uint8_t *out = (uint8_t *)(a.head + L.off_bits);
        const unsigned long long *in8 = (const unsigned long long *)a.bits;
        auto pack8 = [&](int64_t j) -> unsigned long long {
            unsigned long long w;
            if (8 * j + 8 <= nbits) w = in8[j];
            else { w = 0; for (int k = 0; k < 8 && 8 * j + k < nbits; ++k) w |= (unsigned long long)a.bits[8 * j + k] << (8 * k); }
            return ((w & 0x0101010101010101ull) * 0x8040201008040201ull) >> 56;
        };
#if URH_PACK_WORDS
        int64_t ja = j0 + (int64_t)((8 - ((uintptr_t)(out + j0) & 7)) & 7);
        if (ja > j1) ja = j1;
        int64_t nw = (j1 - ja) / 8;
        const int64_t full = nbits / 8;
        if (ja + 8 * nw > full) nw = full > ja ? (full - ja) / 8 : 0;
        for (int64_t k = gtid; k < nw; k += stride) {
            const int64_t j = ja + 8 * k;
            unsigned long long r = 0;
#pragma unroll
            for (int b = 0; b < 8; ++b) r |= (((in8[j + b] & 0x0101010101010101ull) * 0x8040201008040201ull) >> 56) << (8 * b);
            *(unsigned long long *)(out + j) = r;
        }
        for (int64_t j = j0 + gtid; j < ja; j += stride) out[j] = (uint8_t)pack8(j);
        for (int64_t j = ja + 8 * nw + gtid; j < j1; j += stride) out[j] = (uint8_t)pack8(j);
#else
        for (int64_t j = j0 + gtid; j < j1; j += stride) out[j] = (uint8_t)pack8(j);
#endif
    }
    if (a.has_pos && !a.pos_shipped) {
        uint32_t *p32 = (uint32_t *)(a.host + L.off_pos32);
        for (int64_t i = p0 + gtid; i < p1; i += stride) p32[i] = (uint32_t)a.pos[i];
    }
    {
        int64_t *pa = (int64_t *)(a.head + L.off_pauses), *mo = (int64_t *)(a.head + L.off_msg_off), *po = (int64_t *)(a.head + L.off_pos_off);
        if (gtid == 0 && m0 == 0) { mo[0] = 0; po[0] = 0; }
        for (int64_t i = m0 + gtid; i < m1; i += stride) { pa[i] = a.pauses[i]; mo[i + 1] = a.msg_off[i + 1]; po[i + 1] = a.pos_off[i + 1]; }
    }
    int64_t n_esc = 0;
    if (a.esc && a.final) {
        n_esc = a.esc[0];
        const bool over = n_esc > a.esc_cap;
        if (over) n_esc = a.esc_cap;
        int64_t *dst = (int64_t *)(a.head + (a.row16_esc_off > 0 ? a.row16_esc_off : ((L.off_bits + (nbits + 7) / 8 + 15) & ~int64_t(15))));
        if (gtid == 0) dst[0] = over ? -n_esc : n_esc;
        for (int64_t i = gtid; i < n_esc; i += stride) dst[1 + i] = a.esc[1 + i];
    }
    if (a.final && gtid == 0) {
        int64_t *hdr = (int64_t *)a.head;
        const int64_t *c = a.counts;
        const int64_t n_rows = lim(*a.d_n_rows, a.cap_rows);
        hdr[1] = n_rows; hdr[2] = m1; hdr[3] = nbits; hdr[4] = p1; hdr[5] = c[4];
        const bool row16 = a.esc && a.row16_esc_off > 0;
        hdr[6] = URHGPU_BLOB_HEADER_BYTES + n_rows * (row16 ? 2 : (a.esc ? 3 : 5)) + (a.esc ? 8 + n_esc * 8 : 0) + (nbits + 7) / 8 + p1 * 4 + m1 * 24 + 16;
        hdr[7] = a.has_pos | (row16 ? URHGPU_BLOB_ROW16 : (a.esc ? URHGPU_BLOB_LEN16 : 0));
        hdr[8] = L.off_pauses; hdr[9] = L.off_msg_off; hdr[10] = L.off_pos_off; hdr[11] = row16 ? a.row16_esc_off : L.off_row_state; hdr[12] = L.off_bits;
        hdr[13] = L.off_row_len; hdr[14] = L.off_pos32;
        hdr[15] = ((c[1] > a.cap_msg || c[2] > a.cap_bits || (a.has_pos && c[3] > a.cap_pos) || c[4] > a.cap_rows) ? 1 : 0) | (a.seg->err ? 2 : 0);
        hdr[0] = URHGPU_BLOB_MAGIC;
    }
    if (a.final && a.progress && gtid < kMaxSegments) a.progress[gtid * kProgressStride] = 0;
}

int launch_rows_segment(const ResolveArgs &r, const EmitArgs &e, const TileTailMem &m, const BitsParams &bp, SegState *state, const RowsSegment &sg,
                        hipStream_t s) {
    if (r.n_chunks <= 0 || r.local_pass || r.chunk_first != 0 || e.chunk_first != 0 || r.n_local != r.n_chunks || m.n_chunks != r.n_chunks ||
        e.is_ask || m.d_row_base != nullptr || !state || sg.index < 0 || sg.index >= kMaxSegments)
        return URHGPU_ERR_ARG;
    if (sg.c0 < 0 || sg.c0 % kSegAlign || sg.c1 <= sg.c0 || sg.c1 > r.n_chunks || (sg.final ? sg.c1 != r.n_chunks : (sg.c1 % kSegAlign != 0 || sg.c1 >= r.n_chunks)))
        return URHGPU_ERR_ARG;
    static_assert(kSegAlign % kResolveBlock == 0 && kSegAlign % kScanBlock == 0 && kSegAlign % (kTailCPW * kEmitWaves) == 0, "segment alignment");
    if (sg.final && (r.d_n_rows != &state->rows_at[sg.index] || r.d_n_rows_needed != &state->rows_needed)) return URHGPU_ERR_ARG;
    if ((sg.h_state == nullptr) != (sg.h_len == nullptr) || sg.gate.seg != state) return URHGPU_ERR_ARG;
    const TileCarve tc = carve_tile(m);
    EmitTileArgs g;
    g.e = e; g.r = r; g.ft = tc.ft; g.huge = tc.huge; g.huge_cap = kTileHugeCap;
    g.bp = bp; g.ft.want_bits = 1;
    g.w0 = sg.c0 / kTailCPW; g.w_end = sg.final ? tail_waves(r.n_chunks) : sg.c1 / kTailCPW; g.final_seg = sg.final; g.seg = state; g.seg_k = sg.index;
    g.h_state = sg.h_state; g.h_len = sg.h_len;
    g.len16 = (sg.len16 && sg.esc && sg.h_len) ? sg.len16 : 0; g.esc = g.len16 ? sg.esc : nullptr; g.esc_cap = sg.esc_cap;
    g.ft.esc = (g.len16 && sg.index == 0) ? sg.esc : nullptr;
    if (g_tail_skip & 64) { g.h_state = nullptr; g.h_len = nullptr; }
    if (g_tail_skip & 128) g.e.rows = nullptr;
    TileTail ft_resolve = g.ft;
    if (sg.index != 0) ft_resolve.want_bits = 0;
    SegGate gate = sg.gate;
    gate.fused = (sg.fuse_gate && gate.progress && !gate.init && resolve_blocks(sg.c1 - sg.c0) == 1) ? 1 : 0;
    if (!gate.fused && gate.progress) hipLaunchKernelGGL(k_seg_gate, dim3(1), dim3(64), 0, s, gate);
    if (!(g_tail_skip & 1)) hipLaunchKernelGGL(k_resolve_one, dim3((unsigned)resolve_blocks(sg.c1 - sg.c0)), dim3(kResolveBlock), 0, s, r, ft_resolve, sg.c0 / kResolveBlock, gate);
    if (!(g_tail_skip & 2)) hipLaunchKernelGGL(k_emit_rows_tiles, dim3((unsigned)((g.w_end - g.w0 + 1 + kEmitWaves - 1) / kEmitWaves)), dim3(64 * kEmitWaves), 0, s, g);
    return URHGPU_OK;
}

int launch_bits_segment(const TileTailMem &m, const BitsParams &bp, const BitsOut &o, void *scratch, const ScanState &ss, int64_t *rows,
                        int64_t cap_rows, const BitsSegment &sg, const SegPackDst *dst, hipStream_t s) {
    if (m.n_chunks <= 0 || m.d_row_base != nullptr || !sg.state || sg.rows_index < 0 || sg.rows_index >= kMaxSegments) return URHGPU_ERR_ARG;
    if (sg.c0 < 0 || sg.c0 % kSegAlign || sg.c1 <= sg.c0 || sg.c1 > m.n_chunks || (sg.final ? sg.c1 != m.n_chunks : (sg.c1 % kSegAlign != 0 || sg.c1 >= m.n_chunks)))
        return URHGPU_ERR_ARG;
    if (cap_rows <= 0) cap_rows = 1;
    const int64_t cap_desc = tile_desc_cap(cap_rows, m.n_chunks);
    if (ss.desc_bytes < bits_desc_bytes(cap_desc)) return URHGPU_ERR_ARG;
    const TileCarve tc = carve_tile(m);
    const BitsScratch b = carve_bits(scratch, cap_rows);
    SegState *st = sg.state;
    const int64_t *d_n_rows = &st->rows_at[sg.rows_index];
    const int parity = sg.index & 1;
    const int64_t t1 = sg.final ? m.n_chunks + 1 : sg.c1;
    const int64_t cap_groups = cap_rows + 1;
    GranDesc *tdesc = (GranDesc *)m.rdesc + resolve_blocks(m.n_chunks) + 2;
    TileScanArgs ta{rows, d_n_rows, tc.ft.agg, tc.ft.tile_off, tc.ft.tile_cnt, tc.ft.excl, b.groups, cap_groups, &st->n_groups, t1, bp, tdesc,
                    m.epoch, sg.c0 / kScanBlock, st, parity};
    if (!(g_tail_skip & 4)) hipLaunchKernelGGL(k_tile_scan, dim3((unsigned)((t1 - sg.c0 + kScanBlock - 1) / kScanBlock)), dim3(kScanBlock), 0, s, ta);
    ScanDesc<3> *desc3 = (ScanDesc<3> *)((char *)ss.desc + (((size_t)(scan_blocks(cap_desc) + 1) * sizeof(ScanDesc<4>) + 255) & ~size_t(255)));
    GroupLoad gl{b.groups, &st->n_groups, nullptr, sg.final ? 1 : 0, bp.write_pos, sg.final ? 0 : 1};
    const int has_pos = (bp.write_pos && o.pos) ? 1 : 0;
    const int64_t caps[5] = {cap_rows, o.cap_msg, o.cap_bits, o.cap_pos, cap_rows};
    BlobLayout L = blob_layout(caps, cap_rows, o.cap_bits, o.cap_msg, o.cap_pos, has_pos);
    const bool split = dst && dst->host && dst->split;
    if (split) {
        if (!sg.final || sg.c0 != 0) return URHGPU_ERR_ARG;
        const StagedLayout SL = staged_layout(cap_rows, o.cap_bits, o.cap_msg, o.cap_pos, has_pos);
        L.off_row_state = SL.off_row_state; L.off_row_len = SL.off_row_len; L.off_pos32 = SL.off_pos32;
    }
    const bool pos_direct = dst && dst->host && has_pos && sg.final && sg.c0 == 0 && dst->pos_direct;
    uint32_t *h_pos = pos_direct ? (uint32_t *)((char *)dst->host + L.off_pos32) : nullptr;
    GroupStore gs{gl, b.gout, o.msg_off, o.pauses, o.pos_off, o.pos, o.cap_msg, o.cap_pos, h_pos};
    SegGroupLoad sl{gl, st, parity};
    SegGroupStore sst{gs, st, parity};
    SegFinal fin{sl, st, d_n_rows, parity, sg.final ? 1 : 0, BitsCountsFinal{d_n_rows, o.msg_off, o.pos_off, o.counts, b.huge_count, &st->rows_needed, o.h_counts}};
    if (!(g_tail_skip & 8))
        hipLaunchKernelGGL((k_scan_lookback<3, SegGroupLoad, SegGroupStore, SegFinal, kGroupItems>), dim3((unsigned)std::min<int64_t>(scan_grid(b.nbg), 32)),
                           dim3(kScanBlock), 0, s, &st->n_groups_local, sl, desc3, b.nbg, sst, fin, ++*ss.epoch, ss.tickets + 2, 0);
    ExpandTileArgs ea{rows, d_n_rows, tc.ft.excl, tc.ft.tile_off, tc.ft.tile_cnt, b.gout, &st->n_groups, o.bits, o.cap_bits, o.pos, o.cap_pos,
                      bp, tc.huge, m.huge_count, kTileHugeCap, m.parity, t1, sg.c0, h_pos};
    const unsigned tile_blocks = (unsigned)expand_tile_blocks(t1 - sg.c0);
    if (g_tail_skip & 2048) ea.cap_bits = 0;
    if (!(g_tail_skip & 16)) hipLaunchKernelGGL(k_expand_tiles, dim3(tile_blocks + kHugeBlocksX * kHugeBlocksY), dim3(64 * kEmitWaves), 0, s, ea);
    if (dst && dst->host) {
        if (((uintptr_t)o.bits & 7) || ((uintptr_t)dst->host & 15)) return URHGPU_ERR_ARG;
        SegPack pk{o.bits, o.msg_off, o.pauses, o.pos_off, o.pos, o.counts, cap_rows, o.cap_bits, o.cap_msg, o.cap_pos, has_pos, (char *)dst->host,
                   L, st, d_n_rows, parity, sg.final ? 1 : 0, sg.final ? dst->progress_reset : nullptr, pos_direct ? 1 : 0, split ? 1 : 0,
                   (split && dst->host_head) ? (char *)dst->host_head : (char *)dst->host, split ? dst->esc : nullptr, dst->esc_cap,
                   (split && dst->esc) ? dst->row16_esc_off : 0};
        if (dst->cap_host < pk.L.total) return URHGPU_ERR_CAPACITY;
        if (!(g_tail_skip & 32)) hipLaunchKernelGGL(k_pack_seg, dim3(dst->blocks > 0 ? dst->blocks : 32), dim3(256), 0, s, pk);
    }
    return URHGPU_OK;
}

__global__ void k_merge_summary(const int64_t *rows, const int64_t *d_n_rows, int64_t *out5) {
    const int64_t n = *d_n_rows;
    out5[0] = n;
    out5[1] = n ? rows[0] : 0; out5[2] = n ? rows[1] : 0;
    out5[3] = n ? rows[2 * (n - 1)] : 0; out5[4] = n ? rows[2 * (n - 1) + 1] : 0;
}
void launch_merge_summary(const int64_t *rows, const int64_t *d_n_rows, int64_t *d_out5, hipStream_t s) {
    hipLaunchKernelGGL(k_merge_summary, dim3(1), dim3(1), 0, s, rows, d_n_rows, d_out5);
}

__global__ void k_merge_fix(int64_t *rows, const int64_t *d_n_rows, const int64_t *all, int rank, int world, int64_t *d_absorbed) {
    const int64_t n = *d_n_rows;
    *d_absorbed = -1;
    if (n == 0) return;
    auto M = [&](int q, int k) { return all[5 * q + k]; };
    int prev = -1;
    for (int q = rank - 1; q >= 0; --q) if (M(q, 0) > 0) { prev = q; break; }
    const bool absorbed = prev >= 0 && M(prev, 3) == rows[0];
    if (!(absorbed && n == 1)) {
        const int64_t last_state = rows[2 * (n - 1)];
        for (int q = rank + 1; q < world; ++q) {
            if (M(q, 0) == 0) continue;
            if (M(q, 1) != last_state) break;
            rows[2 * (n - 1) + 1] += M(q, 2);
            if (M(q, 0) > 1) break;
        }
    }
    if (absorbed) {
        if (n == 1 && rows[0] == -1) {
            int64_t tot = rows[1];
            for (int q = rank + 1; q < world; ++q) tot += (M(q, 0) > 0) ? M(q, 2) : 0;
            for (int q = rank - 1; q >= 0; --q) {
                if (M(q, 0) == 0) continue;
                tot += M(q, 4);
                if (M(q, 0) > 1) break;
                int pq = -1;
                for (int u = q - 1; u >= 0; --u) if (M(u, 0) > 0) { pq = u; break; }
                if (!(pq >= 0 && M(pq, 3) == M(q, 1))) break;
            }
            *d_absorbed = tot;
        }
        rows[0] = kRowAbsorbed;
    }
}
void launch_merge_fix(int64_t *rows, const int64_t *d_n_rows, const int64_t *d_all, int rank, int world,
                      int64_t *d_absorbed, hipStream_t s) {
    hipLaunchKernelGGL(k_merge_fix, dim3(1), dim3(1), 0, s, rows, d_n_rows, d_all, rank, world, d_absorbed);
// ... 14 lines not shown
```

urh_amd/csrc/runs.hpp:

```cpp
#pragma once
#include <stdint.h>

namespace urh {

constexpr int kBlock = 64;
constexpr int kRows = 16;
constexpr int kRowSamples = kBlock * 2;
constexpr int kTile = kRowSamples * kRows;
constexpr int kSpan = kTile / kBlock;

constexpr uint32_t kStPause = 0;
constexpr uint32_t kStNone = 0xFF;
constexpr int kMaxOrder = 128;
constexpr int kMaxSegments = 16;
constexpr int kProgressStride = 32;

__host__ __device__ inline uint64_t rec_make(int64_t pos, uint32_t st) { return (uint64_t)pos | ((uint64_t)st << 56); }
__host__ __device__ inline int64_t rec_pos(uint64_t r) { return (int64_t)(r & 0x00FFFFFFFFFFFFFFull); }
__host__ __device__ inline uint32_t rec_state(uint64_t r) { return (uint32_t)(r >> 56); }

struct ChunkInfo {
    int64_t pend_pos;
    int64_t lead;
    int64_t start;
    int64_t len;
    int64_t last_pos;
    int32_t cnt;
    uint16_t first_state;
    uint16_t last_state;
    uint16_t pend_state;
    uint16_t init_state;
    int32_t first_acc;
    int32_t pend_acc;
    int32_t pend_stable;
    int32_t pad;
};
static_assert(sizeof(ChunkInfo) == 72, "URHGPU_SHARD_SUMMARY_BYTES (include/urhgpu.h) is sizeof(ChunkInfo)");

}
```

urh_amd/csrc/stream.hip:

```cpp
#include <hip/hip_runtime.h>

#include <algorithm>
#include <new>

#include "common.hpp"
#include "compact.hpp"
#include "launchers.hpp"
#include "pass.hpp"

using namespace urh;

struct urhgpu_stream {
    urhgpu_ctx *ctx = nullptr;
    urhgpu_params p;
    int want_qad = 0, want_pos = 0;
    int64_t n_max = 0, cap_rows = 0, cap_bits = 0, cap_msg = 0, cap_pos = 0, cap_blob = 0;
    struct Slot {
        void *dev = nullptr;
        char *stage = nullptr;
        float *qad = nullptr;
        urhgpu_outputs out;
        char *h_blob2[2] = {nullptr, nullptr};
        char *h_blob = nullptr;
        int64_t *h_counts = nullptr;
        int32_t *h_costas = nullptr;
        hipEvent_t ev_tail = nullptr, ev_copy = nullptr, ev_rows = nullptr, ev_shipped = nullptr;
        int64_t seq = -1, n = 0, copied = 0;
        bool staged = false;
        int64_t copied_rows = 0, copied_pos = 0;
        int state = 0;
        char *d_center = nullptr, *h_center2[2] = {nullptr, nullptr};
        char *d_noise = nullptr, *h_noise2[2] = {nullptr, nullptr};
        char *d_rec = nullptr, *h_rec2[2] = {nullptr, nullptr};
        int64_t *d_rec_pos = nullptr;
    } slot[3];
    int msg_records = 0;
    int64_t rec_divisor = 1, cap_rec = 0;
    int auto_noise = 0;
    int auto_center = 0;
    int64_t center_max_size = -1, center_hist_cap = 0;
    float *qad_ring[4] = {nullptr, nullptr, nullptr, nullptr};
    hipStream_t copy_stream = nullptr;
    int64_t seq = 0;
    int64_t streamed_passes = 0;
    bool len16 = false;
    bool row16_ok = false;
    int64_t esc_extra = 0;
    int64_t last_rows = 0;
    int32_t *h_probe = nullptr;
    int wide_int = 0;
    int64_t wide_passes = 0;
    hipEvent_t ev_probe = nullptr;
    bool probe_pending = false;
    int64_t staged_passes = 0;
    int64_t uploaded_passes = 0;
    int64_t predicted_bytes = 0;
    int64_t predicted_rows = 0, predicted_pos = 0;
    int64_t short_copies = 0;
    bool was_pipelined = false;
    int64_t costas_sum[5] = {0, 0, 0, 0, 0};
};

namespace {

size_t a256(size_t x) { return (x + 255) & ~size_t(255); }

void fill_result(urhgpu_stream *st, urhgpu_stream::Slot &s, urhgpu_host_result *r) {
    memset(r, 0, sizeof(*r));
    if (st->p.mod == URHGPU_MOD_PSK)
        for (int k = 0; k < 5; ++k) st->costas_sum[k] += s.h_costas[k];
    r->seq = s.seq;
    const int64_t *hdr = (const int64_t *)s.h_blob;
    r->n_samples = s.n;
    r->n_rows = hdr[1]; r->n_msg = hdr[2]; r->n_bits = hdr[3]; r->n_pos = hdr[4]; r->rows_needed = hdr[5];
    r->blob_bytes = hdr[6] < 0 ? -hdr[6] : hdr[6];
    r->truncated = (int)hdr[15];
    r->pauses = (const int64_t *)(s.h_blob + hdr[8]);
    r->msg_off = (const int64_t *)(s.h_blob + hdr[9]);
    r->pos_off = (const int64_t *)(s.h_blob + hdr[10]);
    r->row_state = (const int8_t *)(s.h_blob + hdr[11]);
    r->bits_packed = (const uint8_t *)(s.h_blob + hdr[12]);
    r->row_len = (const int32_t *)(s.h_blob + hdr[13]);
    r->row_len16 = nullptr; r->esc = nullptr; r->n_esc = 0; r->row16 = nullptr;
    if (hdr[7] & URHGPU_BLOB_ROW16) {
        r->row_len = nullptr; r->row_state = nullptr;
        r->row16 = (const uint16_t *)(s.h_blob + hdr[13]);
        const int64_t *e = (const int64_t *)(s.h_blob + hdr[11]);
        r->n_esc = e[0] < 0 ? -e[0] : e[0];
        r->esc = e + 1;
    } else if (hdr[7] & URHGPU_BLOB_LEN16) {
        r->row_len = nullptr;
        r->row_len16 = (const uint16_t *)(s.h_blob + hdr[13]);
        const int64_t *e = (const int64_t *)(s.h_blob + ((hdr[12] + (hdr[3] + 7) / 8 + 15) & ~int64_t(15)));
        r->n_esc = e[0] < 0 ? -e[0] : e[0];
        r->esc = e + 1;
    }
    r->pos32 = (hdr[7] & 1) ? (const uint32_t *)(s.h_blob + hdr[14]) : nullptr;
    r->blob = s.h_blob;
    r->d_qad = s.qad;
}

int queue_copy(urhgpu_stream *st, urhgpu_stream::Slot &s) {
    if (s.state != 1) return URHGPU_OK;
    URH_HIP(hipStreamWaitEvent(st->copy_stream, s.ev_tail, 0));
    URH_TRY(launch_pack_blob(&s.out, st->want_pos, st->copy_stream));
    URH_HIP(hipGetLastError());
    int64_t guess = st->predicted_bytes > 0 ? st->predicted_bytes : URHGPU_BLOB_HEADER_BYTES;
    if (guess > st->cap_blob) guess = st->cap_blob;
    URH_HIP(hipMemcpyAsync(s.h_blob, s.out.blob, (size_t)guess, hipMemcpyDeviceToHost, st->copy_stream));
    URH_HIP(hipEventRecord(s.ev_copy, st->copy_stream));
    s.copied = guess;
    s.state = 2;
    return URHGPU_OK;
}

int wait_event(hipEvent_t e) {
    URH_HIP(hipEventSynchronize(e));
    return URHGPU_OK;
}

int finish_copy(urhgpu_stream *st, urhgpu_stream::Slot &s, urhgpu_host_result *r) {
    if (s.state == 1) URH_TRY(queue_copy(st, s));
    if (s.state != 2) return URHGPU_ERR_ARG;
    URH_TRY(wait_event(s.ev_copy));
    if (s.staged) URH_TRY(wait_event(s.ev_shipped));
    const int64_t *hdr = (const int64_t *)s.h_blob;
    if (hdr[0] != URHGPU_BLOB_MAGIC || hdr[6] < 0 || hdr[6] > st->cap_blob) return URHGPU_ERR_ARG;
    if (hdr[15] & 2) {
        snprintf(urh::g_hip_err, sizeof(urh::g_hip_err), "streamed pass %lld: a segment waited 2 s for the hot kernel", (long long)s.seq);
        return URHGPU_ERR_HIP;
    }
    if (s.staged) {
        const StagedLayout SL = staged_layout(st->cap_rows, st->cap_bits, st->cap_msg, st->cap_pos, st->want_pos);
        const int64_t n_rows = hdr[1], n_pos = (hdr[7] & 1) ? hdr[4] : 0;
        const int64_t len_bytes = (hdr[7] & (URHGPU_BLOB_LEN16 | URHGPU_BLOB_ROW16)) ? 2 : 4;
        const bool row16 = (hdr[7] & URHGPU_BLOB_ROW16) != 0;
        const int64_t head = (hdr[12] + (hdr[3] + 7) / 8 + 15) & ~int64_t(15);
        if (n_rows < 0 || n_rows > st->cap_rows || n_pos < 0 || n_pos > st->cap_pos || head < URHGPU_BLOB_HEADER_BYTES || head > SL.head_cap) return URHGPU_ERR_ARG;
        bool more = false;
        auto fetch = [&](int64_t off, int64_t bytes) -> int {
            URH_HIP(hipMemcpyAsync(s.h_blob + off, s.stage + off, (size_t)bytes, hipMemcpyDeviceToHost, st->copy_stream));
            more = true;
            return URHGPU_OK;
        };
        if (head > s.copied) URH_TRY(fetch(s.copied, head - s.copied));
        if (n_rows > s.copied_rows) {
            if (!row16) URH_TRY(fetch(SL.off_row_state + s.copied_rows, n_rows - s.copied_rows));
            URH_TRY(fetch(SL.off_row_len + len_bytes * s.copied_rows, len_bytes * (n_rows - s.copied_rows)));
        }
        if (n_pos > s.copied_pos) URH_TRY(fetch(SL.off_pos32 + 4 * s.copied_pos, 4 * (n_pos - s.copied_pos)));
        if (more) { URH_HIP(hipStreamSynchronize(st->copy_stream)); st->short_copies += 1; }
        st->predicted_rows = n_rows + n_rows / 8 + 4096;
        st->last_rows = n_rows;
        st->predicted_pos = n_pos + n_pos / 8 + 4096;
        fill_result(st, s, r);
        s.state = 3;
        return URHGPU_OK;
    }
    const int64_t total = hdr[6];
    if (total > s.copied) {
        URH_HIP(hipMemcpyAsync(s.h_blob + s.copied, (const char *)s.out.blob + s.copied, (size_t)(total - s.copied), hipMemcpyDeviceToHost,
                               st->copy_stream));
        URH_HIP(hipStreamSynchronize(st->copy_stream));
        st->short_copies += 1;
    }
    st->predicted_bytes = total + total / 8 + 65536;
    fill_result(st, s, r);
    s.state = 3;
    return URHGPU_OK;
}

}

extern "C" {

int urhgpu_stream_capacities(int64_t n_max, const urhgpu_params *p, int64_t *cap_rows, int64_t *cap_bits, int64_t *cap_msg, int64_t *cap_pos) {
    if (!p || n_max <= 0 || p->samples_per_symbol < 1 || p->bits_per_symbol < 1 || p->tolerance < 0) return URHGPU_ERR_ARG;
    const int64_t sps = (int64_t)p->samples_per_symbol;
    const int64_t rows = std::min<int64_t>(n_max / ((int64_t)p->tolerance + 1) + 2, std::max<int64_t>(4096, 4 * (n_max / sps) + 4096));
    const int64_t bits = (n_max / sps + 2 * rows / 8 + 64) * (int64_t)p->bits_per_symbol + rows;
    const int64_t msg = std::max<int64_t>(64, rows / 4);
    if (cap_rows) *cap_rows = rows;
    if (cap_bits) *cap_bits = bits;
    if (cap_msg) *cap_msg = msg;
    if (cap_pos) *cap_pos = bits + 2 * msg + 2;
    return URHGPU_OK;
}

int urhgpu_stream_create(urhgpu_ctx *ctx, int64_t n_max, const urhgpu_params *p, int want_qad, int want_pos, int64_t cap_rows, urhgpu_stream **out) {
    if (!ctx || !p || !out || n_max <= 0 || n_max > INT32_MAX) return URHGPU_ERR_ARG;
    URH_HIP(hipSetDevice(ctx->device));
    urhgpu_stream *st = new (std::nothrow) urhgpu_stream();
    if (!st) return URHGPU_ERR_ARG;
    st->ctx = ctx; st->p = *p; st->want_qad = want_qad ? 1 : 0; st->want_pos = want_pos ? 1 : 0; st->n_max = n_max;
    st->p.write_bit_sample_pos = st->want_pos;
    int status = urhgpu_stream_capacities(n_max, p, &st->cap_rows, &st->cap_bits, &st->cap_msg, &st->cap_pos);
    if (status != URHGPU_OK) { delete st; return status; }
    if (cap_rows > 0) {
        st->cap_rows = cap_rows;
        st->cap_bits = (n_max / (int64_t)p->samples_per_symbol + 2 * cap_rows / 8 + 64) * (int64_t)p->bits_per_symbol + cap_rows;
        st->cap_msg = std::max<int64_t>(64, cap_rows / 4);
        st->cap_pos = st->cap_bits + 2 * st->cap_msg + 2;
    }
    st->cap_blob = blob_capacity(st->cap_rows, st->cap_bits, st->cap_msg, st->cap_pos, st->want_pos);
    {
        const StagedLayout SL = staged_layout(st->cap_rows, st->cap_bits, st->cap_msg, st->cap_pos, st->want_pos);
        st->len16 = SL.head_cap - URHGPU_BLOB_HEADER_BYTES >= 8 + (n_max / 65535 + 2) * 8 + 16;
        st->esc_extra = ((8 + (n_max / 8191 + 2) * 8 + 16 + 255) & ~int64_t(255)) + std::max<int64_t>(0, SL.total - st->cap_blob);
        st->row16_ok = st->len16 && p->bits_per_symbol <= 2;
    }
    if (p->mod == URHGPU_MOD_FSK && (p->dtype == URHGPU_DT_I8 || p->dtype == URHGPU_DT_I16)) {
        if (hipHostMalloc((void **)&st->h_probe, 64) != hipSuccess || hipEventCreateWithFlags(&st->ev_probe, hipEventDisableTiming) != hipSuccess) { delete st; return URHGPU_ERR_HIP; }
        memset(st->h_probe, 0, 64);
    }
    st->was_pipelined = ctx->pipelined;
    if (!ctx->pipelined) { status = urhgpu_ctx_set_pipelined(ctx, 1, nullptr); if (status != URHGPU_OK) { delete st; return status; } }
    status = urhgpu_ctx_reserve(ctx, n_max, p->tolerance);
    if (status == URHGPU_OK && p->mod == URHGPU_MOD_PSK) status = urh::reserve_psk_pass(ctx, n_max, p->tolerance, st->want_qad != 0);
    if (status != URHGPU_OK) { urhgpu_stream_destroy(st); return status; }
    if (hipStreamCreateWithFlags(&st->copy_stream, hipStreamNonBlocking) != hipSuccess) { urhgpu_stream_destroy(st); return URHGPU_ERR_HIP; }
    const size_t b_qad = st->want_qad ? a256((size_t)n_max * 4) : 0, b_rows = a256((size_t)st->cap_rows * 16), b_bits = a256((size_t)st->cap_bits),
                 b_off = a256((size_t)(st->cap_msg + 1) * 8), b_pos = st->want_pos ? a256((size_t)st->cap_pos * 8) : 0, b_blob = a256((size_t)(st->cap_blob + st->esc_extra));
    if (st->want_qad)
        for (auto &q : st->qad_ring)
            if (hipMalloc((void **)&q, b_qad) != hipSuccess) { urhgpu_stream_destroy(st); return URHGPU_ERR_HIP; }
    for (auto &s : st->slot) {
        memset(&s.out, 0, sizeof(s.out));
        if (hipMalloc(&s.dev, b_rows + b_bits + 3 * b_off + b_pos + 256 + 2 * b_blob) != hipSuccess ||
            hipHostMalloc((void **)&s.h_blob2[0], (size_t)(st->cap_blob + st->esc_extra)) != hipSuccess ||
            hipHostMalloc((void **)&s.h_blob2[1], (size_t)(st->cap_blob + st->esc_extra)) != hipSuccess || hipHostMalloc((void **)&s.h_counts, 128) != hipSuccess ||
            hipEventCreateWithFlags(&s.ev_tail, hipEventDisableTiming) != hipSuccess ||
            hipEventCreateWithFlags(&s.ev_copy, hipEventDisableTiming) != hipSuccess ||
            hipEventCreateWithFlags(&s.ev_rows, hipEventDisableTiming) != hipSuccess ||
            hipEventCreateWithFlags(&s.ev_shipped, hipEventDisableTiming) != hipSuccess) {
            urhgpu_stream_destroy(st);
            return URHGPU_ERR_HIP;
        }
        char *d = (char *)s.dev;
        s.out.rows = (int64_t *)d; d += b_rows; s.out.cap_rows = st->cap_rows;
        s.out.bits = (uint8_t *)d; d += b_bits; s.out.cap_bits = st->cap_bits;
        s.out.msg_off = (int64_t *)d; d += b_off;
        s.out.pauses = (int64_t *)d; d += b_off; s.out.cap_msg = st->cap_msg;
        s.out.pos_off = (int64_t *)d; d += b_off;
        if (st->want_pos) { s.out.pos = (int64_t *)d; d += b_pos; s.out.cap_pos = st->cap_pos; }
        s.out.counts = (int64_t *)d; d += 256;
        s.out.blob = d; s.out.cap_blob = st->cap_blob; d += b_blob;
        s.stage = d;
        memset(s.h_counts, 0, 128);
        s.h_costas = (int32_t *)(s.h_counts + 8);
    }
    *out = st;
    return URHGPU_OK;
}

int urhgpu_stream_destroy(urhgpu_stream *st) {
    if (!st) return URHGPU_OK;
    (void)hipSetDevice(st->ctx->device);
    (void)urhgpu_ctx_sync(st->ctx);
    if (st->copy_stream) { (void)hipStreamSynchronize(st->copy_stream); (void)hipStreamDestroy(st->copy_stream); }
    for (auto &s : st->slot) {
        if (s.dev) (void)hipFree(s.dev);
        s.dev = nullptr;
        if (s.h_blob2[0]) (void)hipHostFree(s.h_blob2[0]);
        if (s.h_blob2[1]) (void)hipHostFree(s.h_blob2[1]);
        if (s.h_counts) (void)hipHostFree(s.h_counts);
        if (s.ev_tail) (void)hipEventDestroy(s.ev_tail);
        if (s.ev_copy) (void)hipEventDestroy(s.ev_copy);
        if (s.ev_rows) (void)hipEventDestroy(s.ev_rows);
        if (s.ev_shipped) (void)hipEventDestroy(s.ev_shipped);
    }
    for (auto &s : st->slot) {
        if (s.d_center) (void)hipFree(s.d_center);
        for (char *h : s.h_center2) if (h) (void)hipHostFree(h);
        if (s.d_noise) (void)hipFree(s.d_noise);
        for (char *h : s.h_noise2) if (h) (void)hipHostFree(h);
        if (s.d_rec) (void)hipFree(s.d_rec);
        if (s.d_rec_pos) (void)hipFree(s.d_rec_pos);
        for (char *h : s.h_rec2) if (h) (void)hipHostFree(h);
    }
    for (auto &q : st->qad_ring) if (q) (void)hipFree(q);
    if (st->h_probe) (void)hipHostFree(st->h_probe);
    if (st->ev_probe) (void)hipEventDestroy(st->ev_probe);
    if (!st->was_pipelined) (void)urhgpu_ctx_set_pipelined(st->ctx, 0, nullptr);
    delete st;
    return URHGPU_OK;
}

static int stream_push(urhgpu_stream *st, const void *h_iq, const void *d_iq, int64_t n, urhgpu_host_result *ready);

int urhgpu_stream_set_auto_center(urhgpu_stream *st, int enable, int64_t max_size) {
    if (!st || st->seq != 0) return URHGPU_ERR_ARG;
    if (!enable) { st->auto_center = 0; return URHGPU_OK; }
    if (!st->want_qad) return URHGPU_ERR_ARG;
    urhgpu_ctx *ctx = st->ctx;
    URH_HIP(hipSetDevice(ctx->device));
    urh::CenterScope scope;
    URH_TRY(urh::reserve_auto_center_pass(ctx, st->n_max, st->p.tolerance, st->cap_rows));
    st->center_hist_cap = ctx->tune_center_max_bins;
    const size_t bytes = sizeof(urhgpu_center_result) + (size_t)st->center_hist_cap * 4;
    for (auto &s : st->slot) {
        if (s.d_center) continue;
// ... 63 lines not shown
        if (!st->want_pos) URH_HIP(hipMalloc((void **)&s.d_rec_pos, (size_t)st->cap_pos * 8));
    }
    st->msg_records = 1; st->rec_divisor = message_length_divisor;
    return URHGPU_OK;
}

int urhgpu_stream_msg_records(urhgpu_stream *st, int64_t seq, const urhgpu_msg_record **rec, int64_t *n_msg) {
    if (!st || !st->msg_records || !rec || !n_msg || seq < 0 || seq >= st->seq) return URHGPU_ERR_ARG;
    const urhgpu_stream::Slot &s = st->slot[seq % 3];
    if (!((s.seq == seq && s.state == 3) || (s.seq == seq + 3))) return URHGPU_ERR_ARG;
    const int k = (int)((seq / 3) & 1);
    const int64_t have = ((const int64_t *)s.h_blob2[k])[2];
    if (have > st->cap_rec) return URHGPU_ERR_CAPACITY;
    *rec = (const urhgpu_msg_record *)s.h_rec2[k];
    *n_msg = have < 0 ? 0 : have;
    return URHGPU_OK;
}

int urhgpu_stream_push(urhgpu_stream *st, const void *d_iq, int64_t n, urhgpu_host_result *ready) {
    return stream_push(st, nullptr, d_iq, n, ready);
}

int urhgpu_stream_push_upload(urhgpu_stream *st, const void *h_iq, void *d_iq, int64_t n, urhgpu_host_result *ready) {
    if (!h_iq) return URHGPU_ERR_ARG;
    return stream_push(st, h_iq, d_iq, n, ready);
}

static int stream_push(urhgpu_stream *st, const void *h_iq, const void *d_iq, int64_t n, urhgpu_host_result *ready) {
    if (!st || !d_iq || n <= 2 || n > st->n_max) return URHGPU_ERR_ARG;
    urh::RecordsScope records_scope(st->msg_records != 0);
    urhgpu_ctx *ctx = st->ctx;
    URH_HIP(hipSetDevice(ctx->device));
    const int64_t i = st->seq;
    urhgpu_stream::Slot &s = st->slot[i % 3];
    if (ready) { memset(ready, 0, sizeof(*ready)); ready->seq = -1; }
    if (s.state == 1 || s.state == 2) {
        urhgpu_host_result r;
        URH_TRY(finish_copy(st, s, &r));
        if (ready) *ready = r;
    }
    if (s.state == 3) {
        URH_HIP(hipStreamWaitEvent(ctx->tail_stream, s.ev_copy, 0));
        if (s.staged) URH_HIP(hipStreamWaitEvent(ctx->tail_stream, s.ev_shipped, 0));
    }
    s.state = 0;
    s.h_blob = s.h_blob2[(i / 3) & 1];
    s.qad = st->want_qad ? st->qad_ring[i & 3] : nullptr;
    urhgpu_outputs pass_out = s.out;
    pass_out.qad = s.qad;
    pass_out.blob = nullptr; pass_out.cap_blob = 0;
    pass_out.h_counts = s.h_counts;
    bool streamed = false, staged = false;
    s.staged = false;
    if (st->auto_center || st->auto_noise || st->msg_records) {
        if (h_iq) {
            const size_t bps = st->p.dtype == URHGPU_DT_F32 ? 8 : (st->p.dtype == URHGPU_DT_I16 || st->p.dtype == URHGPU_DT_U16) ? 4 : 2;
            URH_HIP(hipMemcpyAsync(const_cast<void *>(d_iq), h_iq, (size_t)n * bps, hipMemcpyHostToDevice, ctx->stream));
        }
        ctx->costas_stats_next = s.h_costas;
        const bool probe = st->auto_noise && !st->auto_center && st->h_probe != nullptr;
        if (probe) {
            const int permille = ((volatile int32_t *)st->h_probe)[0], pairs = ((volatile int32_t *)st->h_probe)[1];
            if (pairs >= 256) st->wide_int = st->wide_int ? (permille > 3) : (permille >= 10);
            ctx->wide_int_auto = st->wide_int;
            if (st->wide_int) st->wide_passes += 1;
        }
        urhgpu_params pass_p = st->p;
        if (st->msg_records) {
            pass_p.write_bit_sample_pos = 1;
            if (!st->want_pos) { pass_out.pos = s.d_rec_pos; pass_out.cap_pos = st->cap_pos; }
        }
        const int status = urhgpu_iq_to_bits_auto_dev(ctx, d_iq, n, &pass_p, st->auto_noise, st->auto_center, st->center_max_size, &pass_out, s.d_noise,
                                                      st->auto_noise ? s.h_noise2[(i / 3) & 1] : nullptr, s.d_center,
                                                      st->auto_center ? s.h_center2[(i / 3) & 1] : nullptr, st->center_hist_cap);
        ctx->costas_stats_next = nullptr;
        ctx->wide_int_auto = 0;
        URH_TRY(status);
        if (probe) {
            URH_TRY(launch_wide_probe(d_iq, st->p.dtype, n, 0.0f, st->h_probe, ctx->last_tail, &((const urhgpu_noise_result *)s.d_noise)->noise_sqrd));
            URH_HIP(hipEventRecord(st->ev_probe, ctx->last_tail));
            st->probe_pending = true;
        }
        if (st->msg_records)
            URH_TRY(urh::launch_msg_records(d_iq, n, &pass_p, &pass_out, st->rec_divisor, s.d_rec, st->cap_rec, s.h_rec2[(i / 3) & 1], ctx->last_tail));
        URH_HIP(hipEventRecord(s.ev_tail, ctx->last_tail));
        s.state = 1; s.seq = i; s.n = n;
        st->seq = i + 1;
        URH_TRY(queue_copy(st, s));
        return URHGPU_OK;
    }
#ifdef URH_NO_ROW16
    const int len_mode = st->len16 ? 1 : 0;
#else
    const int len_mode = !st->len16 ? 0 : ((st->row16_ok && st->last_rows > n / 64) ? 2 : 1);
#endif
    if (st->h_probe) {
        const int permille = ((volatile int32_t *)st->h_probe)[0], pairs = ((volatile int32_t *)st->h_probe)[1];
#ifndef URH_NO_INT_PROBE
        if (pairs >= 256) st->wide_int = st->wide_int ? (permille > 3) : (permille >= 10);
#endif
        ctx->wide_int_next = st->wide_int;
        if (st->wide_int) st->wide_passes += 1;
    }
    const int pass_status = urh::iq_to_bits_streamed(ctx, d_iq, n, &st->p, &pass_out, s.h_blob, st->cap_blob, s.ev_copy, &streamed, h_iq, s.stage, &staged, s.ev_rows, len_mode);
    ctx->wide_int_next = 0;
    URH_TRY(pass_status);
    if (st->h_probe && streamed) {
        const float nt = st->p.noise_threshold;
        URH_TRY(launch_wide_probe(d_iq, st->p.dtype, n, nt * nt, st->h_probe, ctx->tail_stream));
        URH_HIP(hipEventRecord(st->ev_probe, ctx->tail_stream));
        st->probe_pending = true;
    }
    if (streamed && staged) {
        const StagedLayout SL = staged_layout(st->cap_rows, st->cap_bits, st->cap_msg, st->cap_pos, st->want_pos);
        const int64_t rows = std::min<int64_t>(st->predicted_rows, st->cap_rows), npos = st->want_pos ? std::min<int64_t>(st->predicted_pos, st->cap_pos) : 0;
        const bool skip_copy = (urh::g_tail_skip & 512) != 0;
        if (rows > 0 && !skip_copy) {
            URH_HIP(hipStreamWaitEvent(st->copy_stream, s.ev_rows, 0));
            if (len_mode != 2) URH_HIP(hipMemcpyAsync(s.h_blob + SL.off_row_state, s.stage + SL.off_row_state, (size_t)rows, hipMemcpyDeviceToHost, st->copy_stream));
            URH_HIP(hipMemcpyAsync(s.h_blob + SL.off_row_len, s.stage + SL.off_row_len, (size_t)rows * (len_mode ? 2 : 4), hipMemcpyDeviceToHost, st->copy_stream));
        }
        if (npos > 0 && !skip_copy) {
            URH_HIP(hipStreamWaitEvent(st->copy_stream, s.ev_copy, 0));
            URH_HIP(hipMemcpyAsync(s.h_blob + SL.off_pos32, s.stage + SL.off_pos32, (size_t)npos * 4, hipMemcpyDeviceToHost, st->copy_stream));
        }
        URH_HIP(hipEventRecord(s.ev_shipped, st->copy_stream));
        s.state = 2; s.seq = i; s.n = n; s.copied = SL.head_cap; s.copied_rows = rows; s.copied_pos = npos; s.staged = true;
        st->seq = i + 1;
        st->staged_passes += 1;
        return URHGPU_OK;
    }
    if (streamed) {
        s.state = 2; s.seq = i; s.n = n; s.copied = st->cap_blob;
        st->seq = i + 1;
        st->streamed_passes += 1;
        if (h_iq) st->uploaded_passes += 1;
        return URHGPU_OK;
    }
    if (h_iq) {
        const size_t bps = st->p.dtype == URHGPU_DT_F32 ? 8 : (st->p.dtype == URHGPU_DT_I16 || st->p.dtype == URHGPU_DT_U16) ? 4 : 2;
        URH_HIP(hipMemcpyAsync(const_cast<void *>(d_iq), h_iq, (size_t)n * bps, hipMemcpyHostToDevice, ctx->stream));
    }
    ctx->costas_stats_next = s.h_costas;
    const int ordinary_status = urhgpu_iq_to_bits_dev(ctx, d_iq, n, &st->p, &pass_out);
    ctx->costas_stats_next = nullptr;
    URH_TRY(ordinary_status);
    URH_HIP(hipEventRecord(s.ev_tail, ctx->last_tail));
    s.state = 1; s.seq = i; s.n = n;
    st->seq = i + 1;
    URH_TRY(queue_copy(st, s));
    return URHGPU_OK;
}

int urhgpu_stream_wide_passes(urhgpu_stream *st, int64_t *n_passes) {
    if (!st || !n_passes) return URHGPU_ERR_ARG;
    *n_passes = st->wide_passes;
    return URHGPU_OK;
}

int urhgpu_stream_stats(urhgpu_stream *st, int64_t *out4) {
    if (!st || !out4) return URHGPU_ERR_ARG;
    out4[0] = st->seq; out4[1] = st->short_copies; out4[2] = st->predicted_bytes; out4[3] = st->cap_blob;
    if (st->streamed_passes + st->staged_passes > 0) out4[2] = -(st->streamed_passes + st->staged_passes);
    return URHGPU_OK;
}

int urhgpu_stream_costas_stats(urhgpu_stream *st, int64_t *out5) {
    if (!st || !out5) return URHGPU_ERR_ARG;
    for (int k = 0; k < 5; ++k) out5[k] = st->costas_sum[k];
    return URHGPU_OK;
}

int urhgpu_stream_flush(urhgpu_stream *st, urhgpu_host_result *out3, int *n_out) {
    if (!st || !out3 || !n_out) return URHGPU_ERR_ARG;
    URH_HIP(hipSetDevice(st->ctx->device));
    *n_out = 0;
    int order[3] = {0, 1, 2};
    std::sort(order, order + 3, [&](int a, int b) { return st->slot[a].seq < st->slot[b].seq; });
    for (int k = 0; k < 3; ++k) {
        urhgpu_stream::Slot &s = st->slot[order[k]];
// ... 12 lines not shown
```

urh_amd/csrc/stream_pass.hip:

```cpp
#include "pass.hpp"

namespace urh {

static int segment_bounds(int64_t n_chunks, int wanted, int shape, int last_units, int64_t *bound ) {
    const int64_t blocks = n_chunks / kSegAlign;
    int S = wanted;
    if (S > kMaxSegments) S = kMaxSegments;
    if (S > blocks) S = (int)blocks;
    if (S < 1) S = 1;
    bound[0] = 0;
    if (shape == 1 && S > 2) {
        int64_t left = blocks, at = 0;
        for (int k = 0; k < S - 1; ++k) {
            int64_t take = left / 2;
            const int64_t must_leave = S - 1 - k;
            if (take < 1) take = 1;
            if (left - take < must_leave) take = left - must_leave;
            at += take; left -= take;
            bound[k + 1] = at * kSegAlign;
        }
    } else if (shape == 2 && S > 1) {
        int64_t last = last_units < 1 ? 1 : last_units;
        if (last > blocks - (S - 1)) last = blocks - (S - 1);
        const int64_t rest = blocks - last;
        for (int k = 1; k < S; ++k) bound[k] = (rest * k / (S - 1)) * kSegAlign;
    } else {
        for (int k = 1; k < S; ++k) bound[k] = (blocks * k / S) * kSegAlign;
    }
    bound[S] = n_chunks;
    for (int k = 0; k < S; ++k)
        if (bound[k + 1] <= bound[k]) return 0;
    return S;
}

namespace {
struct StreamPass {
    urhgpu_ctx *ctx; const void *d_iq; int64_t n; const urhgpu_params *p; const urhgpu_outputs *out;
    const void *h_iq;
    void *host_blob; int64_t cap_host;
    void *real_host_blob;
    Plan pl; RunArgs a;
    int S; int64_t bound[kMaxSegments + 1]; uint32_t target[kMaxSegments];
    bool direct, to_stage;
    BitsParams bp; int has_pos; BlobLayout host_layout;
    int slot; uint32_t *progress; SegState *st;
    hipStream_t s; hipEvent_t hot_done;
    ChunkInfo *chunks; uint64_t *slab; void *rs_mem, *scratch; TileTailMem tm; ScanState ss;
    int policy(void *stage_blob);
    int begin();
    int hot();
    int tail(hipEvent_t ev_ready, hipEvent_t ev_rows, int len16);
};
}

int StreamPass::policy(void *stage_blob) {
    S = 0;
    int segs = runs_streamable(a) ? segment_bounds(pl.n_chunks, h_iq ? ctx->tune_upload_pieces : ctx->tune_stream_segments, h_iq ? 2 : 0, 1, bound) : 0;
    int policy = ctx->tune_stream_policy;
    if (policy == 5) policy = (p->write_bit_sample_pos && out->pos && !ctx->tune_stream_pos_direct) ? 0 : (ctx->tune_stream_latency ? 4 : (stage_blob ? 6 : 3));
    if (policy == 6 && !stage_blob) policy = 3;
    direct = to_stage = false;
    if (!h_iq && runs_streamable(a) && host_blob && (policy == 3 || policy == 6)) { direct = true; to_stage = (policy == 6); }
    if (segs < 2 && !direct) return URHGPU_OK;
    if (policy == 2 && !h_iq) return URHGPU_OK;
    if ((policy == 0 || policy == 4) && ctx->passes_begun > 0 && !h_iq) {
        const hipError_t q = hipEventQuery(ctx->ev_tail[(ctx->flip + 2) % 3]);
        if (q == hipErrorNotReady) {
            (void)hipGetLastError();
            if (policy == 0 || !host_blob) return URHGPU_OK;
            direct = true; to_stage = (stage_blob != nullptr);
        } else if (q != hipSuccess) URH_HIP(q);
    }
    S = segs;
    if (direct) { S = 1; bound[0] = 0; bound[1] = pl.n_chunks; }
    real_host_blob = host_blob;
    if (to_stage) host_blob = stage_blob;
    return URHGPU_OK;
}

static int stream_resources(urhgpu_ctx *ctx) {
    if (ctx->d_seg) return URHGPU_OK;
    URH_HIP(hipMalloc(&ctx->d_seg, 3 * kSegBlockBytes));
    URH_HIP(hipMemset(ctx->d_seg, 0, 3 * kSegBlockBytes));
    URH_HIP(hipDeviceSynchronize());
    URH_HIP(hipStreamCreateWithFlags(&ctx->bits_stream, hipStreamNonBlocking));
    for (int k = 0; k < kMaxSegments; ++k) URH_HIP(hipEventCreateWithFlags(&ctx->ev_piece[k], hipEventDisableTiming));
    for (int k = 0; k < 3; ++k) {
        URH_HIP(hipEventCreateWithFlags(&ctx->ev_hot_done[k], hipEventDisableTiming));
        URH_HIP(hipEventCreateWithFlags(&ctx->ev_bits[k], hipEventDisableTiming));
        for (int j = 0; j < kMaxSegments; ++j) URH_HIP(hipEventCreateWithFlags(&ctx->ev_rows[k][j], hipEventDisableTiming));
    }
    return URHGPU_OK;
}

int StreamPass::begin() {
    URH_TRY(stream_resources(ctx));
    bp = bits_params(p);
    has_pos = (bp.write_pos && out->pos) ? 1 : 0;
    memset(&host_layout, 0, sizeof(host_layout));
    if (host_blob) {
        const int64_t caps[5] = {out->cap_rows, out->cap_msg, out->cap_bits, out->cap_pos, out->cap_rows};
        host_layout = blob_layout(caps, out->cap_rows, out->cap_bits, out->cap_msg, out->cap_pos, has_pos);
        if (cap_host < host_layout.total) return URHGPU_ERR_CAPACITY;
    }
    URH_TRY(begin_pipelined_pass(ctx));
    slot = ctx->flip;
    progress = (uint32_t *)((char *)ctx->d_seg + (size_t)slot * kSegBlockBytes);
    st = (SegState *)((char *)progress + kMaxSegments * kProgressStride * 4);
    static_assert(kMaxSegments * kProgressStride * 4 + sizeof(SegState) <= kSegBlockBytes && kMaxSegments <= 16, "segment block");
    if (ctx->seg_dirty[slot]) {
        URH_HIP(hipDeviceSynchronize());
        URH_HIP(hipMemset(progress, 0, kSegBlockBytes));
        URH_HIP(hipDeviceSynchronize());
        ctx->seg_dirty[slot] = false;
    }
    URH_TRY(ctx->arena.reserve(digitize_scratch_bytes(pl, out->cap_rows, false, true)));
    ctx->arena.reset();
    ctx->seg_dirty[slot] = true;
    s = ctx->stream;
    URH_TRY(hot_stream_begin(ctx, &s));
    chunks = (ChunkInfo *)ctx->arena.take((size_t)pl.n_chunks * sizeof(ChunkInfo));
    slab = (uint64_t *)ctx->arena.take((size_t)pl.n_chunks * pl.slab_stride * 8);
    rs_mem = ctx->arena.take(resolve_scratch_bytes(pl.n_chunks));
    if (!chunks || !slab || !rs_mem) return URHGPU_ERR_ARG;
    a.chunks = chunks; a.slab = slab;
    URH_TRY(tile_tail_mem(ctx, pl.n_chunks, true, &tm));
    const int64_t cap = std::max<int64_t>(out->cap_rows, 1);
    scratch = ctx->arena.take(bits_scratch_bytes(cap));
    if (!scratch) return URHGPU_ERR_ARG;
    URH_TRY(scan_state(ctx, tile_desc_cap(cap, pl.n_chunks), &ss));
    a.progress = progress; a.n_seg = S;
    for (int k = 0; k < S; ++k) {
        const int64_t hi = (k < S - 1) ? bound[k + 1] + 1 : pl.n_chunks, lo = (k == 0) ? 0 : bound[k] + 1;
        a.seg_end[k] = (int32_t)hi;
        target[k] = (uint32_t)(hi - lo);
    }
    return URHGPU_OK;
}

int StreamPass::hot() {
    if (h_iq) {
        a.progress = nullptr; a.n_seg = 0;
        const size_t bps = (size_t)dtype_bytes(p->dtype);
        int64_t piece_lo[kMaxSegments], piece_hi[kMaxSegments];
        for (int k = 0; k < S; ++k) {
            piece_lo[k] = k == 0 ? 0 : piece_hi[k - 1];
            piece_hi[k] = (k < S - 1) ? std::min<int64_t>(bound[k + 1] + 1, pl.n_chunks) : pl.n_chunks;
        }
        hipStream_t up = s;
        for (int k = 0; k < S; ++k) {
            {
                const int64_t s0 = piece_lo[k] * pl.chunk_len, s1 = std::min<int64_t>(piece_hi[k] * pl.chunk_len, n);
                URH_HIP(hipMemcpyAsync((char *)const_cast<void *>(d_iq) + (size_t)s0 * bps, (const char *)h_iq + (size_t)s0 * bps, (size_t)(s1 - s0) * bps,
                                       hipMemcpyHostToDevice, up));
            }
            a.launch_lo = piece_lo[k]; a.launch_hi = piece_hi[k];
            const int stl = launch_demod_runs_iq(a, p->dtype, p->mod, out->qad != nullptr, s);
            if (stl != URHGPU_OK) return stl;
            URH_HIP(hipEventRecord(ctx->ev_piece[k], s));
        }
        a.launch_lo = 0; a.launch_hi = 0;
        URH_HIP(hipEventRecord(ctx->ev_hot_done[slot], s));
        hot_done = ctx->ev_hot_done[slot];
        return URHGPU_OK;
    }
    if (direct) { a.progress = nullptr; a.n_seg = 0; }
    return hot_launch(ctx, a, p, true, s, true, ctx->ev_hot_done[slot], nullptr, &hot_done);
}

int StreamPass::tail(hipEvent_t ev_ready, hipEvent_t ev_rows, int len16) {
    const bool event_start = (h_iq != nullptr) || direct;
    hipStream_t ts = ctx->tail_stream, tb = ctx->bits_stream;
    ResolveArgs r;
    EmitArgs e;
    table_args(ctx, p, pl, n, chunks, slab, rs_mem, out->rows, out->cap_rows, &st->n_acc, &st->rows_at[S - 1], &st->rows_needed, false, &r, &e);
    int8_t *h_state = nullptr; int32_t *h_len = nullptr;
    BitsOut bo{out->bits, out->cap_bits, out->msg_off, out->pauses, out->cap_msg, out->pos, out->cap_pos, out->pos_off, out->counts, out->h_counts};
    if (host_blob) { h_state = (int8_t *)((char *)host_blob + host_layout.off_row_state); h_len = (int32_t *)((char *)host_blob + host_layout.off_row_len); }
    if (to_stage) {
        const StagedLayout SL = staged_layout(out->cap_rows, out->cap_bits, out->cap_msg, out->cap_pos, has_pos);
        h_state = (int8_t *)((char *)host_blob + SL.off_row_state); h_len = (int32_t *)((char *)host_blob + SL.off_row_len);
    }
    const bool l16 = to_stage && len16 != 0;
    const bool row16 = l16 && len16 == 2;
    int64_t row16_esc_off = 0;
    if (row16) row16_esc_off = staged_layout(out->cap_rows, out->cap_bits, out->cap_msg, out->cap_pos, has_pos).total;
    int64_t *esc = l16 ? (int64_t *)((char *)host_blob + (row16 ? row16_esc_off : (int64_t)URHGPU_BLOB_HEADER_BYTES)) : nullptr;
    const int64_t esc_cap = row16 ? n / 8191 + 2 : n / 65535 + 2;
    SegPackDst dst{host_blob, cap_host, progress, 0, (direct && ctx->tune_stream_pos_direct) ? 1 : 0, to_stage ? 1 : 0, to_stage ? real_host_blob : nullptr,
                   esc, esc_cap, row16_esc_off};
    int Sb = h_iq ? S : 1;
    int bits_end_at[kMaxSegments];
    for (int j = 0; j < Sb - 1; ++j) bits_end_at[j] = (int)((int64_t)(S - 1) * (j + 1) / (Sb - 1)) - 1;
    bits_end_at[Sb - 1] = S - 1;
    int jb = 0;
    int64_t bits_from = 0;
    for (int k = 0; k < S; ++k) {
        if (h_iq) URH_HIP(hipStreamWaitEvent(ts, ctx->ev_piece[k], 0));
        else if (direct) URH_HIP(hipStreamWaitEvent(ts, hot_done, 0));
        RowsSegment sg{k, k == S - 1 ? 1 : 0, bound[k], bound[k + 1], SegGate{event_start ? nullptr : progress, k, target[k], k == 0 ? 1 : 0, st, (long long)200000000, 0},
                       h_state, h_len, 1, l16 ? (row16 ? 2 : 1) : 0, esc, esc_cap};
        URH_TRY(launch_rows_segment(r, e, tm, bp, st, sg, ts));
        if (to_stage && ev_rows) URH_HIP(hipEventRecord(ev_rows, ts));
        while (jb < Sb && bits_end_at[jb] < k) ++jb;
        if (jb < Sb && bits_end_at[jb] == k) {
            const bool last = (jb == Sb - 1);
            BitsSegment bs{jb, last ? 1 : 0, bits_from, bound[k + 1], k, st};
            if (last) {
                if (jb > 0) {
                    URH_HIP(hipEventRecord(ctx->ev_bits[slot], tb));
                    URH_HIP(hipStreamWaitEvent(ts, ctx->ev_bits[slot], 0));
                }
                URH_TRY(launch_bits_segment(tm, bp, bo, scratch, ss, out->rows, out->cap_rows, bs, &dst, ts));
            } else {
                URH_HIP(hipEventRecord(ctx->ev_rows[slot][jb], ts));
                URH_HIP(hipStreamWaitEvent(tb, ctx->ev_rows[slot][jb], 0));
                URH_TRY(launch_bits_segment(tm, bp, bo, scratch, ss, out->rows, out->cap_rows, bs, &dst, tb));
            }
            bits_from = bound[k + 1];
            ++jb;
        }
    }
    URH_HIP(hipGetLastError());
    if (!host_blob) URH_HIP(hipMemsetAsync(progress, 0, kMaxSegments * kProgressStride * 4, ts));
    ctx->seg_dirty[slot] = false;
    if (ev_ready) URH_HIP(hipEventRecord(ev_ready, ts));
    URH_HIP(hipStreamWaitEvent(ts, hot_done, 0));
    if (s != ctx->stream && ctx->stream != nullptr) URH_HIP(hipStreamWaitEvent(ctx->stream, hot_done, 0));
    URH_TRY(end_pipelined_pass(ctx));
    return URHGPU_OK;
}

int iq_to_bits_streamed(urhgpu_ctx *ctx, const void *d_iq, int64_t n, const urhgpu_params *p, const urhgpu_outputs *out, void *host_blob,
                        int64_t cap_host, hipEvent_t ev_ready, bool *streamed, const void *h_iq, void *stage_blob, bool *staged, hipEvent_t ev_rows, int len16) {
    *streamed = false;
    if (staged) *staged = false;
    if (!ctx || !p || !out || n <= 0 || !d_iq || !out->rows || !out->counts) return URHGPU_ERR_ARG;
    if (dtype_bytes(p->dtype) == 0) return URHGPU_ERR_DTYPE;
    const bool want_bits = out->bits && out->msg_off && out->pauses && out->pos_off;
    if (!ctx->pipelined || !ctx->tail_stream || n <= 2 || p->mod == URHGPU_MOD_PSK || p->mod == URHGPU_MOD_ASK || !g_tile_tail || !want_bits ||
        (ctx->tune_stream_segments < 2 && !h_iq) || out->cap_rows < 1)
        return URHGPU_OK;
    URH_TRY(check_params(p, true));
    if (((uintptr_t)d_iq & 15) || (out->qad && ((uintptr_t)out->qad & 7))) return URHGPU_ERR_ARG;
    URH_HIP(hipSetDevice(ctx->device));
    StreamPass sp;
    sp.ctx = ctx; sp.d_iq = d_iq; sp.n = n; sp.p = p; sp.out = out; sp.h_iq = h_iq; sp.host_blob = host_blob; sp.cap_host = cap_host;
    sp.pl = make_plan(ctx, n, p->tolerance);
    URH_TRY(hot_run_args(ctx, p, sp.pl, n, 0, true, &sp.a));
    sp.a.in = d_iq; sp.a.qad = out->qad;
    sp.a.lds_pad = ctx->hot_lds_pad;
    if (ctx->wide_int_next) sp.a.wide_int = 1;
    URH_TRY(sp.policy(stage_blob));
    if (sp.S == 0) return URHGPU_OK;
    if (sp.to_stage && staged) *staged = true;
    URH_TRY(sp.begin());
    URH_TRY(sp.hot());
    URH_TRY(sp.tail(ev_ready, ev_rows, len16));
    *streamed = true;
    return URHGPU_OK;
}

}
```

Before: 487,400.

## Ship staged row segments to host per segment using ticketed progress counters

The hot kernel now signals segment progress through per-64-chunk ticket counters, so only the last finisher of each group bumps the segment progress atomic. This cuts contention on the shared counter. The tail writes per-segment row counts into pinned host memory and records per-segment events, which lets the stream copy predicted row ranges to the host while later segments are still running and refetch any mispredicted ranges afterwards. The default segment count drops from 7 to 4. The cost is extra ticket buffers, resets of those buffers, and more complex copy bookkeeping that could issue extra small copies.

```diff
diff --git a/include/urhgpu.h b/include/urhgpu.h
--- a/include/urhgpu.h
+++ b/include/urhgpu.h
@@ -292,6 +292,8 @@
                           int load_kind);
 int urhgpu_test_hot_stamps(int on);
 int urhgpu_test_tail_skip(int mask);
+int urhgpu_test_seg_copy_plan(int points, const int64_t *pred_at, int64_t pred_total, int64_t cap_rows, const int64_t *actual_at, int64_t n_rows,
+                              int64_t *hi_out, int64_t *refetch_out, int *n_refetch);
 int urhgpu_test_fetch_chunk_tables(urhgpu_ctx *ctx, void *host_dst, int64_t n_chunks);
 int urhgpu_memcpy_to_host(urhgpu_ctx *ctx, const void *d_src, void *host_dst, int64_t bytes);
 int urhgpu_memcpy_dtod(urhgpu_ctx *ctx, void *d_dst, const void *d_src, int64_t bytes);
diff --git a/urh_amd/_lib.py b/urh_amd/_lib.py
--- a/urh_amd/_lib.py
+++ b/urh_amd/_lib.py
@@ -171,6 +171,7 @@
     "urhgpu_test_hot_probe": (_i, [_vp, _vp, _i64, C.POINTER(Params), _vp, _i, _i, _i, _i, _i, _vp, C.POINTER(_i64), _vp, _vp, _i, _i]),
     "urhgpu_test_hot_stamps": (_i, [_i]),
     "urhgpu_test_tail_skip": (_i, [_i]),
+    "urhgpu_test_seg_copy_plan": (_i, [_i, _vp, _i64, _i64, _vp, _i64, _vp, _vp, _vp]),
     "urhgpu_test_fetch_chunk_tables": (_i, [_vp, _vp, _i64]),
     "urhgpu_test_fast_division_dev": (_i, [_vp, C.c_uint64, _i, C.POINTER(C.c_uint64)]),
     "urhgpu_test_sincosf_fast_dev": (_i, [_vp, C.POINTER(C.c_uint64)]),
diff --git a/urh_amd/csrc/common.hpp b/urh_amd/csrc/common.hpp
--- a/urh_amd/csrc/common.hpp
+++ b/urh_amd/csrc/common.hpp
@@ -127,7 +127,10 @@
     int tile_parity = 0;
     void *d_seg = nullptr;
     bool seg_dirty[3] = {false, false, false};
-    int tune_stream_segments = 7;
+    void *d_seg_tickets = nullptr;
+    int64_t seg_ticket_cap = 0;
+    int tune_stream_ship_stride = 1;
+    int tune_stream_segments = 4;
     int tune_stream_policy = 5;
     long long passes_begun = 0;
     bool tune_stream_latency = false;
@@ -150,9 +153,17 @@
 constexpr size_t kSegBlockBytes = 4096;
 
 namespace urh {
+struct SegShip {
+    int64_t *h_rows_at = nullptr;
+    int points = 0;
+    int seg[16];
+    hipEvent_t ev[16];
+    int64_t bound[16 + 1];
+    int n_seg = 0;
+};
 int iq_to_bits_streamed(urhgpu_ctx *ctx, const void *d_iq, int64_t n, const urhgpu_params *p, const urhgpu_outputs *out, void *host_blob,
                         int64_t cap_host, hipEvent_t ev_ready, bool *streamed, const void *h_iq, void *stage_blob = nullptr, bool *staged = nullptr,
-                        hipEvent_t ev_rows = nullptr, int len16 = 0);
+                        hipEvent_t ev_rows = nullptr, int len16 = 0, SegShip *ship = nullptr);
 hipError_t wait_stream(const urhgpu_ctx *ctx, hipStream_t s);
 int reserve_psk_pass(urhgpu_ctx *ctx, int64_t n_max, int tolerance, bool want_qad);
 int join_tail(urhgpu_ctx *ctx);
diff --git a/urh_amd/csrc/compact.hpp b/urh_amd/csrc/compact.hpp
--- a/urh_amd/csrc/compact.hpp
+++ b/urh_amd/csrc/compact.hpp
@@ -47,6 +47,40 @@
     return S;
 }
 
+inline void seg_copy_plan(int points, const int64_t *pred_at, int64_t pred_total, int64_t cap_rows, int64_t *hi) {
+    int64_t prev = 0, prev_pred = 0;
+    for (int k = 0; k < points; ++k) {
+        int64_t h = 0;
+        if (k == points - 1) h = pred_total;
+        else if (pred_at) {
+            const int64_t seg = pred_at[k] > prev_pred ? pred_at[k] - prev_pred : 0;
+            h = pred_at[k] - seg / 8 - 1024;
+            prev_pred = pred_at[k] > prev_pred ? pred_at[k] : prev_pred;
+        }
+        if (h > cap_rows) h = cap_rows;
+        if (h < prev) h = prev;
+        hi[k] = h; prev = h;
+    }
+}
+inline int seg_copy_refetch(int points, const int64_t *hi, const int64_t *actual_at, int64_t n_rows, int64_t *r_lo, int64_t *r_hi) {
+    int m = 0;
+    auto push = [&](int64_t a, int64_t b) {
+        if (b > n_rows) b = n_rows;
+        if (a < 0) a = 0;
+        if (a >= b) return;
+        if (m > 0 && r_hi[m - 1] == a) r_hi[m - 1] = b;
+        else { r_lo[m] = a; r_hi[m] = b; ++m; }
+    };
+    int64_t lo = 0;
+    for (int k = 0; k < points - 1; ++k) {
+        const int64_t valid_to = actual_at[k] < lo ? lo : (actual_at[k] < hi[k] ? actual_at[k] : hi[k]);
+        push(valid_to, hi[k]);
+        lo = hi[k];
+    }
+    if (points > 0) push(hi[points - 1], n_rows);
+    return m;
+}
+
 inline int64_t blob_capacity(int64_t cap_rows, int64_t cap_bits, int64_t cap_msg, int64_t cap_pos, int has_pos) {
     const int64_t c[5] = {cap_rows, cap_msg, cap_bits, cap_pos, cap_rows};
     return blob_layout(c, cap_rows, cap_bits, cap_msg, cap_pos, has_pos).total;
diff --git a/urh_amd/csrc/ctx.hip b/urh_amd/csrc/ctx.hip
--- a/urh_amd/csrc/ctx.hip
+++ b/urh_amd/csrc/ctx.hip
@@ -134,6 +134,7 @@
     if (ctx->own_tail_stream && ctx->tail_stream) (void)hipStreamDestroy(ctx->tail_stream);
     if (ctx->d_seg) {
         (void)hipFree(ctx->d_seg);
+        if (ctx->d_seg_tickets) (void)hipFree(ctx->d_seg_tickets);
         if (ctx->bits_stream) { (void)hipStreamSynchronize(ctx->bits_stream); (void)hipStreamDestroy(ctx->bits_stream); }
         for (hipEvent_t e : ctx->ev_piece) if (e) (void)hipEventDestroy(e);
         for (int k = 0; k < 3; ++k) {
@@ -220,6 +221,7 @@
     else if (!strcmp(key, "stream_segments")) { if (value < 1 || value > kMaxSegments) return URHGPU_ERR_ARG; ctx->tune_stream_segments = value; }
     else if (!strcmp(key, "stream_policy")) { if (value < 0 || value > 6) return URHGPU_ERR_ARG; ctx->tune_stream_policy = value; }
     else if (!strcmp(key, "stream_latency")) { ctx->tune_stream_latency = value != 0; }
+    else if (!strcmp(key, "stream_ship_stride")) { if (value < 1 || value > kMaxSegments) return URHGPU_ERR_ARG; ctx->tune_stream_ship_stride = value; }
     else if (!strcmp(key, "stream_pos_direct")) { ctx->tune_stream_pos_direct = value != 0; }
     else if (!strcmp(key, "spin_wait")) { ctx->tune_spin_wait = value != 0; }
     else if (!strcmp(key, "shard_summary_generic")) { ctx->tune_shard_summary_generic = value != 0; }
diff --git a/urh_amd/csrc/demod_runs.hip b/urh_amd/csrc/demod_runs.hip
--- a/urh_amd/csrc/demod_runs.hip
+++ b/urh_amd/csrc/demod_runs.hip
@@ -1425,10 +1425,16 @@
     }
     if (through) {
         __asm__ volatile("s_waitcnt vmcnt(0)" ::: "memory");
-        if (lane == 0) {
-            int k = 0;
-            while (k < p.n_seg - 1 && chunk >= (int64_t)p.seg_end[k]) ++k;
-            __hip_atomic_fetch_add(p.progress + k * kProgressStride, 1u, __ATOMIC_RELAXED, __HIP_MEMORY_SCOPE_AGENT);
+        if (lane == 0 && p.n_seg > 0) {
+            const int64_t grp = chunk / kTicketChunks;
+            const int64_t left = (int64_t)p.n_count - grp * kTicketChunks;
+            const uint32_t size = left < kTicketChunks ? (uint32_t)left : (uint32_t)kTicketChunks;
+            const uint32_t before = __hip_atomic_fetch_add(p.tickets + grp * kTicketStride, 1u, __ATOMIC_RELAXED, __HIP_MEMORY_SCOPE_AGENT);
+            if (before + 1 == size) {
+                int k = 0;
+                while (k < p.n_seg - 1 && grp >= (int64_t)p.seg_end[k]) ++k;
+                __hip_atomic_fetch_add(p.progress + k * kProgressStride, 1u, __ATOMIC_RELAXED, __HIP_MEMORY_SCOPE_AGENT);
+            }
         }
     }
 }
diff --git a/urh_amd/csrc/launchers.hpp b/urh_amd/csrc/launchers.hpp
--- a/urh_amd/csrc/launchers.hpp
+++ b/urh_amd/csrc/launchers.hpp
@@ -31,7 +31,9 @@
     float dm_noise_sqrd, dm_max_magnitude, dm_noise_val;
     int lds_pad;
     uint32_t *progress;
+    uint32_t *tickets;
     int32_t n_seg;
+    int32_t n_count;
     int32_t seg_end[kMaxSegments];
     int64_t launch_lo, launch_hi;
     int64_t graded_from, graded_len;
@@ -230,6 +232,7 @@
     int len16;
     int64_t *esc;
     int64_t esc_cap;
+    int64_t *h_rows_at = nullptr;
 };
 struct BitsSegment {
     int index;
@@ -249,6 +252,8 @@
     const int64_t *esc;
     int64_t esc_cap;
     int64_t row16_esc_off;
+    uint32_t *tickets_reset = nullptr;
+    int64_t n_tickets = 0;
 };
 
 struct TileTailMem {
diff --git a/urh_amd/csrc/probes.hip b/urh_amd/csrc/probes.hip
--- a/urh_amd/csrc/probes.hip
+++ b/urh_amd/csrc/probes.hip
@@ -92,6 +92,20 @@
 
 int urhgpu_test_hot_stamps(int on) { urh::g_stamp_probe = (on != 0); return URHGPU_OK; }
 int urhgpu_test_tail_skip(int mask) { urh::g_tail_skip = mask; return URHGPU_OK; }
+
+int urhgpu_test_seg_copy_plan(int points, const int64_t *pred_at, int64_t pred_total, int64_t cap_rows, const int64_t *actual_at, int64_t n_rows,
+                              int64_t *hi_out, int64_t *refetch_out, int *n_refetch) {
+    if (points < 1 || points > kMaxSegments || cap_rows < 0 || !hi_out || (actual_at && (!refetch_out || !n_refetch || n_rows < 0))) return URHGPU_ERR_ARG;
+    urh::seg_copy_plan(points, pred_at, pred_total, cap_rows, hi_out);
+    if (n_refetch) *n_refetch = 0;
+    if (actual_at) {
+        int64_t lo[kMaxSegments + 1], hi[kMaxSegments + 1];
+        const int m = urh::seg_copy_refetch(points, hi_out, actual_at, n_rows, lo, hi);
+        for (int i = 0; i < m; ++i) { refetch_out[2 * i] = lo[i]; refetch_out[2 * i + 1] = hi[i]; }
+        *n_refetch = m;
+    }
+    return URHGPU_OK;
+}
 
 int urhgpu_test_fetch_chunk_tables(urhgpu_ctx *ctx, void *host_dst, int64_t n_chunks) {
     if (!ctx || !host_dst || n_chunks < 1) return URHGPU_ERR_ARG;
diff --git a/urh_amd/csrc/pulse_table.hip b/urh_amd/csrc/pulse_table.hip
--- a/urh_amd/csrc/pulse_table.hip
+++ b/urh_amd/csrc/pulse_table.hip
@@ -923,6 +923,7 @@
     int len16;
     int64_t *esc;
     int64_t esc_cap;
+    int64_t *h_rows_at;
 };
 
 __host__ __device__ static inline int64_t tail_waves(int64_t n_items) { return (n_items + kTailCPW - 1) / kTailCPW; }
@@ -985,7 +986,11 @@
     if (totals) {
         const ResElem pre = base;
         if (!g.final_seg) {
-            if (lane == 0) g.seg->rows_at[g.seg_k] = (r.rows != nullptr && pre.cnt > r.cap_rows) ? r.cap_rows : pre.cnt;
+            if (lane == 0) {
+                const int64_t final_rows = (r.rows != nullptr && pre.cnt > r.cap_rows) ? r.cap_rows : pre.cnt;
+                g.seg->rows_at[g.seg_k] = final_rows;
+                if (g.h_rows_at) g.h_rows_at[g.seg_k] = final_rows;
+            }
             return;
         }
         const int64_t c = r.n_chunks;
@@ -1644,7 +1649,7 @@
     memset(&g.bp, 0, sizeof(g.bp));
     if (bp) { g.bp = *bp; g.ft.want_bits = 1; }
     const unsigned gb = (unsigned)resolve_blocks(r.n_chunks);
-    g.w0 = 0; g.w_end = tail_waves(r.n_chunks); g.final_seg = 1; g.seg = nullptr; g.seg_k = 0; g.h_state = nullptr; g.h_len = nullptr; g.len16 = 0; g.esc = nullptr; g.esc_cap = 0; g.ft.esc = nullptr;
+    g.w0 = 0; g.w_end = tail_waves(r.n_chunks); g.final_seg = 1; g.seg = nullptr; g.seg_k = 0; g.h_state = nullptr; g.h_len = nullptr; g.len16 = 0; g.esc = nullptr; g.esc_cap = 0; g.ft.esc = nullptr; g.h_rows_at = nullptr;
     SegGate no_gate;
     memset(&no_gate, 0, sizeof(no_gate));
     if (!(g_tail_skip & 1)) hipLaunchKernelGGL(k_resolve_one, dim3(gb), dim3(kResolveBlock), 0, s, r, g.ft, (int64_t)0, no_gate);
@@ -1796,6 +1801,8 @@
     const int64_t *esc;
     int64_t esc_cap;
     int64_t row16_esc_off;
+    uint32_t *tickets;
+    int64_t n_tickets;
 };
 __global__ __launch_bounds__(256) void k_pack_seg(const SegPack a) {
     URH_TAIL_PRIO();
@@ -1872,6 +1879,8 @@
         hdr[0] = URHGPU_BLOB_MAGIC;
     }
     if (a.final && a.progress && gtid < kMaxSegments) a.progress[gtid * kProgressStride] = 0;
+    if (a.final && a.progress && a.tickets)
+        for (int64_t i = gtid; i < a.n_tickets; i += stride) a.tickets[i * kTicketStride] = 0;
 }
 
 int launch_rows_segment(const ResolveArgs &r, const EmitArgs &e, const TileTailMem &m, const BitsParams &bp, SegState *state, const RowsSegment &sg,
@@ -1889,7 +1898,7 @@
     g.e = e; g.r = r; g.ft = tc.ft; g.huge = tc.huge; g.huge_cap = kTileHugeCap;
     g.bp = bp; g.ft.want_bits = 1;
     g.w0 = sg.c0 / kTailCPW; g.w_end = sg.final ? tail_waves(r.n_chunks) : sg.c1 / kTailCPW; g.final_seg = sg.final; g.seg = state; g.seg_k = sg.index;
-    g.h_state = sg.h_state; g.h_len = sg.h_len;
+    g.h_state = sg.h_state; g.h_len = sg.h_len; g.h_rows_at = sg.h_rows_at;
     g.len16 = (sg.len16 && sg.esc && sg.h_len) ? sg.len16 : 0; g.esc = g.len16 ? sg.esc : nullptr; g.esc_cap = sg.esc_cap;
     g.ft.esc = (g.len16 && sg.index == 0) ? sg.esc : nullptr;
     if (g_tail_skip & 64) { g.h_state = nullptr; g.h_len = nullptr; }
@@ -1953,7 +1962,7 @@
         SegPack pk{o.bits, o.msg_off, o.pauses, o.pos_off, o.pos, o.counts, cap_rows, o.cap_bits, o.cap_msg, o.cap_pos, has_pos, (char *)dst->host,
                    L, st, d_n_rows, parity, sg.final ? 1 : 0, sg.final ? dst->progress_reset : nullptr, pos_direct ? 1 : 0, split ? 1 : 0,
                    (split && dst->host_head) ? (char *)dst->host_head : (char *)dst->host, split ? dst->esc : nullptr, dst->esc_cap,
-                   (split && dst->esc) ? dst->row16_esc_off : 0};
+                   (split && dst->esc) ? dst->row16_esc_off : 0, sg.final ? dst->tickets_reset : nullptr, dst->n_tickets};
         if (dst->cap_host < pk.L.total) return URHGPU_ERR_CAPACITY;
         if (!(g_tail_skip & 32)) hipLaunchKernelGGL(k_pack_seg, dim3(dst->blocks > 0 ? dst->blocks : 32), dim3(256), 0, s, pk);
     }
diff --git a/urh_amd/csrc/runs.hpp b/urh_amd/csrc/runs.hpp
--- a/urh_amd/csrc/runs.hpp
+++ b/urh_amd/csrc/runs.hpp
@@ -14,6 +14,8 @@
 constexpr int kMaxOrder = 128;
 constexpr int kMaxSegments = 16;
 constexpr int kProgressStride = 32;
+constexpr int kTicketChunks = 64;
+constexpr int kTicketStride = 32;
 
 __host__ __device__ inline uint64_t rec_make(int64_t pos, uint32_t st) { return (uint64_t)pos | ((uint64_t)st << 56); }
 __host__ __device__ inline int64_t rec_pos(uint64_t r) { return (int64_t)(r & 0x00FFFFFFFFFFFFFFull); }
diff --git a/urh_amd/csrc/stream.hip b/urh_amd/csrc/stream.hip
--- a/urh_amd/csrc/stream.hip
+++ b/urh_amd/csrc/stream.hip
@@ -28,6 +28,9 @@
         int64_t seq = -1, n = 0, copied = 0;
         bool staged = false;
         int64_t copied_rows = 0, copied_pos = 0;
+        int seg_points = 0, seg_n = 0;
+        int seg_at[kMaxSegments];
+        int64_t seg_hi[kMaxSegments], seg_bound[kMaxSegments + 1];
         int state = 0;
         char *d_center = nullptr, *h_center2[2] = {nullptr, nullptr};
         char *d_noise = nullptr, *h_noise2[2] = {nullptr, nullptr};
@@ -57,6 +60,8 @@
     int64_t predicted_bytes = 0;
     int64_t predicted_rows = 0, predicted_pos = 0;
     int64_t short_copies = 0;
+    int pred_n_seg = 0;
+    int64_t pred_n = 0, pred_at[kMaxSegments], pred_bound[kMaxSegments + 1];
     bool was_pipelined = false;
     int64_t costas_sum[5] = {0, 0, 0, 0, 0};
 };
@@ -64,6 +69,8 @@
 namespace {
 
 size_t a256(size_t x) { return (x + 255) & ~size_t(255); }
+constexpr int kRowsAtWord = 16;
+constexpr size_t kCountsBytes = (size_t)(kRowsAtWord + kMaxSegments) * 8;
 
 void fill_result(urhgpu_stream *st, urhgpu_stream::Slot &s, urhgpu_host_result *r) {
     memset(r, 0, sizeof(*r));
@@ -144,10 +151,20 @@
             return URHGPU_OK;
         };
         if (head > s.copied) URH_TRY(fetch(s.copied, head - s.copied));
-        if (n_rows > s.copied_rows) {
-            if (!row16) URH_TRY(fetch(SL.off_row_state + s.copied_rows, n_rows - s.copied_rows));
-            URH_TRY(fetch(SL.off_row_len + len_bytes * s.copied_rows, len_bytes * (n_rows - s.copied_rows)));
-        }
+        auto fetch_rows = [&](int64_t from, int64_t to) -> int {
+            if (!row16) URH_TRY(fetch(SL.off_row_state + from, to - from));
+            URH_TRY(fetch(SL.off_row_len + len_bytes * from, len_bytes * (to - from)));
+            return URHGPU_OK;
+        };
+        if (s.seg_points > 0) {
+            int64_t at[kMaxSegments], r_lo[kMaxSegments + 1], r_hi[kMaxSegments + 1];
+            for (int k = 0; k < s.seg_points - 1; ++k) at[k] = s.h_counts[kRowsAtWord + s.seg_at[k]];
+            const int m = seg_copy_refetch(s.seg_points, s.seg_hi, at, n_rows, r_lo, r_hi);
+            for (int i = 0; i < m; ++i) URH_TRY(fetch_rows(r_lo[i], r_hi[i]));
+            st->pred_n_seg = s.seg_n; st->pred_n = s.n;
+            for (int j = 0; j <= s.seg_n; ++j) st->pred_bound[j] = s.seg_bound[j];
+            for (int j = 0; j < s.seg_n; ++j) st->pred_at[j] = (j < s.seg_n - 1) ? std::min(std::max<int64_t>(s.h_counts[kRowsAtWord + j], 0), n_rows) : n_rows;
+        } else if (n_rows > s.copied_rows) URH_TRY(fetch_rows(s.copied_rows, n_rows));
         if (n_pos > s.copied_pos) URH_TRY(fetch(SL.off_pos32 + 4 * s.copied_pos, 4 * (n_pos - s.copied_pos)));
         if (more) { URH_HIP(hipStreamSynchronize(st->copy_stream)); st->short_copies += 1; }
         st->predicted_rows = n_rows + n_rows / 8 + 4096;
@@ -228,7 +245,7 @@
         memset(&s.out, 0, sizeof(s.out));
         if (hipMalloc(&s.dev, b_rows + b_bits + 3 * b_off + b_pos + 256 + 2 * b_blob) != hipSuccess ||
             hipHostMalloc((void **)&s.h_blob2[0], (size_t)(st->cap_blob + st->esc_extra)) != hipSuccess ||
-            hipHostMalloc((void **)&s.h_blob2[1], (size_t)(st->cap_blob + st->esc_extra)) != hipSuccess || hipHostMalloc((void **)&s.h_counts, 128) != hipSuccess ||
+            hipHostMalloc((void **)&s.h_blob2[1], (size_t)(st->cap_blob + st->esc_extra)) != hipSuccess || hipHostMalloc((void **)&s.h_counts, kCountsBytes) != hipSuccess ||
             hipEventCreateWithFlags(&s.ev_tail, hipEventDisableTiming) != hipSuccess ||
             hipEventCreateWithFlags(&s.ev_copy, hipEventDisableTiming) != hipSuccess ||
             hipEventCreateWithFlags(&s.ev_rows, hipEventDisableTiming) != hipSuccess ||
@@ -246,7 +263,7 @@
         s.out.counts = (int64_t *)d; d += 256;
         s.out.blob = d; s.out.cap_blob = st->cap_blob; d += b_blob;
         s.stage = d;
-        memset(s.h_counts, 0, 128);
+        memset(s.h_counts, 0, kCountsBytes);
         s.h_costas = (int32_t *)(s.h_counts + 8);
     }
     *out = st;
@@ -416,6 +433,9 @@
     pass_out.h_counts = s.h_counts;
     bool streamed = false, staged = false;
     s.staged = false;
+    s.seg_points = 0;
+    urh::SegShip ship;
+    ship.h_rows_at = s.h_counts + kRowsAtWord;
     if (st->auto_center || st->auto_noise || st->msg_records) {
         if (h_iq) {
             const size_t bps = st->p.dtype == URHGPU_DT_F32 ? 8 : (st->p.dtype == URHGPU_DT_I16 || st->p.dtype == URHGPU_DT_U16) ? 4 : 2;
@@ -466,7 +486,7 @@
         ctx->wide_int_next = st->wide_int;
         if (st->wide_int) st->wide_passes += 1;
     }
-    const int pass_status = urh::iq_to_bits_streamed(ctx, d_iq, n, &st->p, &pass_out, s.h_blob, st->cap_blob, s.ev_copy, &streamed, h_iq, s.stage, &staged, s.ev_rows, len_mode);
+    const int pass_status = urh::iq_to_bits_streamed(ctx, d_iq, n, &st->p, &pass_out, s.h_blob, st->cap_blob, s.ev_copy, &streamed, h_iq, s.stage, &staged, s.ev_rows, len_mode, &ship);
     ctx->wide_int_next = 0;
     URH_TRY(pass_status);
     if (st->h_probe && streamed) {
@@ -479,7 +499,30 @@
         const StagedLayout SL = staged_layout(st->cap_rows, st->cap_bits, st->cap_msg, st->cap_pos, st->want_pos);
         const int64_t rows = std::min<int64_t>(st->predicted_rows, st->cap_rows), npos = st->want_pos ? std::min<int64_t>(st->predicted_pos, st->cap_pos) : 0;
         const bool skip_copy = (urh::g_tail_skip & 512) != 0;
-        if (rows > 0 && !skip_copy) {
+        int64_t copied_rows = rows;
+        if (ship.points > 0) {
+            const int64_t *pred = nullptr;
+            int64_t pred_pts[kMaxSegments];
+            bool same_cut = st->pred_n_seg == ship.n_seg && st->pred_n == n;
+            for (int j = 0; same_cut && j <= ship.n_seg; ++j) same_cut = st->pred_bound[j] == ship.bound[j];
+            if (same_cut) { for (int k = 0; k < ship.points; ++k) pred_pts[k] = st->pred_at[ship.seg[k]]; pred = pred_pts; }
+            seg_copy_plan(ship.points, pred, rows, st->cap_rows, s.seg_hi);
+            int64_t lo = 0;
+            for (int k = 0; k < ship.points; ++k) {
+                s.seg_at[k] = ship.seg[k];
+                const int64_t hi = s.seg_hi[k];
+                if (hi > lo && !skip_copy) {
+                    URH_HIP(hipStreamWaitEvent(st->copy_stream, ship.ev[k], 0));
+                    if (len_mode != 2) URH_HIP(hipMemcpyAsync(s.h_blob + SL.off_row_state + lo, s.stage + SL.off_row_state + lo, (size_t)(hi - lo), hipMemcpyDeviceToHost, st->copy_stream));
+                    const int64_t lb = len_mode ? 2 : 4;
+                    URH_HIP(hipMemcpyAsync(s.h_blob + SL.off_row_len + lb * lo, s.stage + SL.off_row_len + lb * lo, (size_t)((hi - lo) * lb), hipMemcpyDeviceToHost, st->copy_stream));
+                }
+                lo = hi;
+            }
+            s.seg_points = ship.points; s.seg_n = ship.n_seg;
+            for (int j = 0; j <= ship.n_seg; ++j) s.seg_bound[j] = ship.bound[j];
+            copied_rows = lo;
+        } else if (rows > 0 && !skip_copy) {
             URH_HIP(hipStreamWaitEvent(st->copy_stream, s.ev_rows, 0));
             if (len_mode != 2) URH_HIP(hipMemcpyAsync(s.h_blob + SL.off_row_state, s.stage + SL.off_row_state, (size_t)rows, hipMemcpyDeviceToHost, st->copy_stream));
             URH_HIP(hipMemcpyAsync(s.h_blob + SL.off_row_len, s.stage + SL.off_row_len, (size_t)rows * (len_mode ? 2 : 4), hipMemcpyDeviceToHost, st->copy_stream));
@@ -489,7 +532,7 @@
             URH_HIP(hipMemcpyAsync(s.h_blob + SL.off_pos32, s.stage + SL.off_pos32, (size_t)npos * 4, hipMemcpyDeviceToHost, st->copy_stream));
         }
         URH_HIP(hipEventRecord(s.ev_shipped, st->copy_stream));
-        s.state = 2; s.seq = i; s.n = n; s.copied = SL.head_cap; s.copied_rows = rows; s.copied_pos = npos; s.staged = true;
+        s.state = 2; s.seq = i; s.n = n; s.copied = SL.head_cap; s.copied_rows = copied_rows; s.copied_pos = npos; s.staged = true;
         st->seq = i + 1;
         st->staged_passes += 1;
         return URHGPU_OK;
diff --git a/urh_amd/csrc/stream_pass.hip b/urh_amd/csrc/stream_pass.hip
--- a/urh_amd/csrc/stream_pass.hip
+++ b/urh_amd/csrc/stream_pass.hip
@@ -44,6 +44,8 @@
     bool direct, to_stage;
     BitsParams bp; int has_pos; BlobLayout host_layout;
     int slot; uint32_t *progress; SegState *st;
+    uint32_t *tickets; int64_t n_tickets;
+    SegShip *ship; bool seg_staged;
     hipStream_t s; hipEvent_t hot_done;
     ChunkInfo *chunks; uint64_t *slab; void *rs_mem, *scratch; TileTailMem tm; ScanState ss;
     int policy(void *stage_blob);
@@ -73,6 +75,8 @@
     }
     S = segs;
     if (direct) { S = 1; bound[0] = 0; bound[1] = pl.n_chunks; }
+    seg_staged = !direct && !h_iq && S >= 2 && stage_blob && host_blob && ship;
+    if (seg_staged) to_stage = true;
     real_host_blob = host_blob;
     if (to_stage) host_blob = stage_blob;
     return URHGPU_OK;
@@ -93,8 +97,23 @@
     return URHGPU_OK;
 }
 
+static int ticket_resources(urhgpu_ctx *ctx, int64_t n_tickets) {
+    if (ctx->seg_ticket_cap >= n_tickets) return URHGPU_OK;
+    const int64_t cap = std::max<int64_t>(n_tickets + n_tickets / 4, 256);
+    URH_HIP(hipDeviceSynchronize());
+    if (ctx->d_seg_tickets) { URH_HIP(hipFree(ctx->d_seg_tickets)); ctx->d_seg_tickets = nullptr; ctx->seg_ticket_cap = 0; }
+    const size_t bytes = (size_t)3 * cap * kTicketStride * 4;
+    URH_HIP(hipMalloc(&ctx->d_seg_tickets, bytes));
+    URH_HIP(hipMemset(ctx->d_seg_tickets, 0, bytes));
+    URH_HIP(hipDeviceSynchronize());
+    ctx->seg_ticket_cap = cap;
+    return URHGPU_OK;
+}
+
 int StreamPass::begin() {
     URH_TRY(stream_resources(ctx));
+    n_tickets = (pl.n_chunks + kTicketChunks - 1) / kTicketChunks;
+    URH_TRY(ticket_resources(ctx, n_tickets));
     bp = bits_params(p);
     has_pos = (bp.write_pos && out->pos) ? 1 : 0;
     memset(&host_layout, 0, sizeof(host_layout));
@@ -107,10 +126,12 @@
     slot = ctx->flip;
     progress = (uint32_t *)((char *)ctx->d_seg + (size_t)slot * kSegBlockBytes);
     st = (SegState *)((char *)progress + kMaxSegments * kProgressStride * 4);
+    tickets = (uint32_t *)ctx->d_seg_tickets + (size_t)slot * ctx->seg_ticket_cap * kTicketStride;
     static_assert(kMaxSegments * kProgressStride * 4 + sizeof(SegState) <= kSegBlockBytes && kMaxSegments <= 16, "segment block");
     if (ctx->seg_dirty[slot]) {
         URH_HIP(hipDeviceSynchronize());
         URH_HIP(hipMemset(progress, 0, kSegBlockBytes));
+        URH_HIP(hipMemset(tickets, 0, (size_t)ctx->seg_ticket_cap * kTicketStride * 4));
         URH_HIP(hipDeviceSynchronize());
         ctx->seg_dirty[slot] = false;
     }
@@ -129,11 +150,13 @@
     scratch = ctx->arena.take(bits_scratch_bytes(cap));
     if (!scratch) return URHGPU_ERR_ARG;
     URH_TRY(scan_state(ctx, tile_desc_cap(cap, pl.n_chunks), &ss));
-    a.progress = progress; a.n_seg = S;
+    static_assert(kSegAlign % kTicketChunks == 0, "segment boundaries start a ticket group");
+    static_assert(kMaxSegments == 16, "SegShip's arrays (common.hpp)");
+    a.progress = progress; a.tickets = tickets; a.n_seg = S; a.n_count = (int32_t)pl.n_chunks;
     for (int k = 0; k < S; ++k) {
-        const int64_t hi = (k < S - 1) ? bound[k + 1] + 1 : pl.n_chunks, lo = (k == 0) ? 0 : bound[k] + 1;
+        const int64_t hi = (k < S - 1) ? bound[k + 1] / kTicketChunks + 1 : n_tickets, lo = (k == 0) ? 0 : bound[k] / kTicketChunks + 1;
         a.seg_end[k] = (int32_t)hi;
-        target[k] = (uint32_t)(hi - lo);
+        target[k] = (uint32_t)(hi > lo ? hi - lo : 0);
     }
     return URHGPU_OK;
 }
@@ -165,6 +188,7 @@
         return URHGPU_OK;
     }
     if (direct) { a.progress = nullptr; a.n_seg = 0; }
+    if (direct && (g_tail_skip & 4096)) { a.progress = progress; a.n_seg = (g_tail_skip & 8192) ? 0 : 1; }
     return hot_launch(ctx, a, p, true, s, true, ctx->ev_hot_done[slot], nullptr, &hot_done);
 }
 
@@ -188,7 +212,9 @@
     int64_t *esc = l16 ? (int64_t *)((char *)host_blob + (row16 ? row16_esc_off : (int64_t)URHGPU_BLOB_HEADER_BYTES)) : nullptr;
     const int64_t esc_cap = row16 ? n / 8191 + 2 : n / 65535 + 2;
     SegPackDst dst{host_blob, cap_host, progress, 0, (direct && ctx->tune_stream_pos_direct) ? 1 : 0, to_stage ? 1 : 0, to_stage ? real_host_blob : nullptr,
-                   esc, esc_cap, row16_esc_off};
+                   esc, esc_cap, row16_esc_off, tickets, n_tickets};
+    if (ship) { ship->points = 0; ship->n_seg = S; for (int k = 0; k <= S; ++k) ship->bound[k] = bound[k]; }
+    const int ship_stride = ctx->tune_stream_ship_stride < 1 ? 1 : ctx->tune_stream_ship_stride;
     int Sb = h_iq ? S : 1;
     int bits_end_at[kMaxSegments];
     for (int j = 0; j < Sb - 1; ++j) bits_end_at[j] = (int)((int64_t)(S - 1) * (j + 1) / (Sb - 1)) - 1;
@@ -199,9 +225,14 @@
         if (h_iq) URH_HIP(hipStreamWaitEvent(ts, ctx->ev_piece[k], 0));
         else if (direct) URH_HIP(hipStreamWaitEvent(ts, hot_done, 0));
         RowsSegment sg{k, k == S - 1 ? 1 : 0, bound[k], bound[k + 1], SegGate{event_start ? nullptr : progress, k, target[k], k == 0 ? 1 : 0, st, (long long)200000000, 0},
-                       h_state, h_len, 1, l16 ? (row16 ? 2 : 1) : 0, esc, esc_cap};
+                       h_state, h_len, 1, l16 ? (row16 ? 2 : 1) : 0, esc, esc_cap, seg_staged ? ship->h_rows_at : nullptr};
         URH_TRY(launch_rows_segment(r, e, tm, bp, st, sg, ts));
-        if (to_stage && ev_rows) URH_HIP(hipEventRecord(ev_rows, ts));
+        if (to_stage && !seg_staged && ev_rows) URH_HIP(hipEventRecord(ev_rows, ts));
+        if (seg_staged && (k == S - 1 || (k + 1) % ship_stride == 0)) {
+            hipEvent_t ev = ctx->ev_rows[slot][k];
+            URH_HIP(hipEventRecord(ev, ts));
+            ship->seg[ship->points] = k; ship->ev[ship->points] = ev; ship->points += 1;
+        }
         while (jb < Sb && bits_end_at[jb] < k) ++jb;
         if (jb < Sb && bits_end_at[jb] == k) {
             const bool last = (jb == Sb - 1);
@@ -222,7 +253,10 @@
         }
     }
     URH_HIP(hipGetLastError());
-    if (!host_blob) URH_HIP(hipMemsetAsync(progress, 0, kMaxSegments * kProgressStride * 4, ts));
+    if (!host_blob) {
+        URH_HIP(hipMemsetAsync(progress, 0, kMaxSegments * kProgressStride * 4, ts));
+        URH_HIP(hipMemsetAsync(tickets, 0, (size_t)n_tickets * kTicketStride * 4, ts));
+    }
     ctx->seg_dirty[slot] = false;
     if (ev_ready) URH_HIP(hipEventRecord(ev_ready, ts));
     URH_HIP(hipStreamWaitEvent(ts, hot_done, 0));
@@ -232,9 +266,11 @@
 }
 
 int iq_to_bits_streamed(urhgpu_ctx *ctx, const void *d_iq, int64_t n, const urhgpu_params *p, const urhgpu_outputs *out, void *host_blob,
-                        int64_t cap_host, hipEvent_t ev_ready, bool *streamed, const void *h_iq, void *stage_blob, bool *staged, hipEvent_t ev_rows, int len16) {
+                        int64_t cap_host, hipEvent_t ev_ready, bool *streamed, const void *h_iq, void *stage_blob, bool *staged, hipEvent_t ev_rows, int len16,
+                        SegShip *ship) {
     *streamed = false;
     if (staged) *staged = false;
+    if (ship) { ship->points = 0; ship->n_seg = 0; }
     if (!ctx || !p || !out || n <= 0 || !d_iq || !out->rows || !out->counts) return URHGPU_ERR_ARG;
     if (dtype_bytes(p->dtype) == 0) return URHGPU_ERR_DTYPE;
     const bool want_bits = out->bits && out->msg_off && out->pauses && out->pos_off;
@@ -245,6 +281,7 @@
     if (((uintptr_t)d_iq & 15) || (out->qad && ((uintptr_t)out->qad & 7))) return URHGPU_ERR_ARG;
     URH_HIP(hipSetDevice(ctx->device));
     StreamPass sp;
+    sp.ship = (ship && ship->h_rows_at) ? ship : nullptr; sp.seg_staged = false; sp.tickets = nullptr; sp.n_tickets = 0;
     sp.ctx = ctx; sp.d_iq = d_iq; sp.n = n; sp.p = p; sp.out = out; sp.h_iq = h_iq; sp.host_blob = host_blob; sp.cap_host = cap_host;
     sp.pl = make_plan(ctx, n, p->tolerance);
     URH_TRY(hot_run_args(ctx, p, sp.pl, n, 0, true, &sp.a));
```

Result: no change. 484,500 (-0.6%).
